# zhirui-gao/PoseProbe

Hardware: AMD Instinct MI355X
Metric: rays_per_sec_train_step (higher is better)
Workload: dtype f32 (3xf16-split products); 1 GPU; DTU-scan1-like 3-view 400x400, object-branch train step (ray select, render, losses, backward, TV+Adam), 160^3 grid, 186 samples/ray, N_rand=1024/GPU; per-step ray permutation + jitter pre-generated on the host and resident in HBM (the reference draws randperm inside the step); grid=160, n_rand_per_gpu=1024, samples_in_bbox_last_step=57637, parallelism=single GPU

## Files before the change

### poseprobe_amd/_lib.py

```python
import ctypes
import os
import re

HERE = os.path.dirname(os.path.abspath(__file__))
HEADER = os.path.join(HERE, '..', 'include', 'poseprobe_hip.h')
SO_PATH = os.path.join(HERE, 'libposeprobe_hip.so')


class pp_scene(ctypes.Structure):
    _fields_ = [('xyz_min', ctypes.c_float * 3), ('xyz_max', ctypes.c_float * 3), ('size', ctypes.c_int32 * 3),
                ('voxel_size', ctypes.c_float), ('stepsize', ctypes.c_float), ('near_clip', ctypes.c_float),
                ('far_clip', ctypes.c_float), ('bg', ctypes.c_float), ('n_samples', ctypes.c_int32),
                ('out_range', ctypes.c_float), ('k0_dim', ctypes.c_int32), ('pos_pe', ctypes.c_int32),
                ('view_pe', ctypes.c_int32), ('sdf_index_exact', ctypes.c_int32)]


def parse_header(path=HEADER):
    text = open(path).read()
    text = re.sub(r'/\*.*?\*/', '', text, flags=re.S)
    protos = {}
    for m in re.finditer(r'\bint\s+(pp_\w+)\s*\(([^;]*?)\)\s*;', text, flags=re.S):
        name, args = m.group(1), m.group(2)
        parsed = []
        for a in args.split(','):
            a = ' '.join(a.split())
            if a in ('void', ''):
                continue
            argname = re.findall(r'(\w+)$', a)[0]
            if 'pp_scene' in a:
                ct = ctypes.POINTER(pp_scene)
            elif 'char*' in a.replace(' *', '*'):
                ct = ctypes.c_char_p
            elif '*' in a:
                ct = ctypes.c_void_p
            elif 'uint8_t' in a and '*' not in a:
                ct = ctypes.c_uint8
            elif 'int64_t' in a:
                ct = ctypes.c_int64
            elif 'int32_t' in a or a.startswith('int '):
                ct = ctypes.c_int32
            elif 'float' in a:
                ct = ctypes.c_float
            else:
                raise ValueError(f'unhandled argument "{a}" in {name}')
            parsed.append((ct, argname))
        protos[name] = parsed
    return protos


class PoseProbeError(RuntimeError):
    pass


_lib = None


def lib():
    global _lib
    if _lib is not None:
        return _lib
    if not os.path.exists(SO_PATH):
        raise PoseProbeError(f'{SO_PATH} is missing: run `python -m poseprobe_amd.build_ext` '
                             '(there is no CPU / eager fallback for the hot path)')
    L = ctypes.CDLL(SO_PATH)
    L.pp_last_error.restype = ctypes.c_char_p
    L.pp_abi_version.restype = ctypes.c_int
    want = header_abi_version()
    if L.pp_abi_version() != want:
        raise PoseProbeError(f'{SO_PATH} reports ABI {L.pp_abi_version()}, include/poseprobe_hip.h declares {want}: '
                             'rebuild with `python -m poseprobe_amd.build_ext`')
    for name, args in parse_header().items():
        fn = getattr(L, name)
        fn.restype = ctypes.c_int
        fn.argtypes = [ct for ct, _ in args]
    _lib = L
    return L


def header_abi_version(path=HEADER):
    return int(re.search(r'#define\s+PP_ABI_VERSION\s+(\d+)', open(path).read()).group(1))


OPTION_NAMES = ('mlp_fused', 'grid_chunks', 'nerf_split', 'mlp_split', 'mlp_wgs', 'nerf_chain', 'nerf_chain_nw',
                'nerf_chain_head', 'mlp_pack', 'warp_lean')


class Context:

    def __init__(self, **options):
        self.handle = ctypes.c_void_p()
        check(lib().pp_context_create(ctypes.byref(self.handle)), 'pp_context_create')
        for k, v in options.items():
            self.set(k, v)

    def set(self, name, value):
        check(lib().pp_context_set_option(self.handle, name.encode(), int(value)), 'pp_context_set_option')

    def get(self, name):
        v = ctypes.c_int32()
        check(lib().pp_context_get_option(self.handle, name.encode(), ctypes.byref(v)), 'pp_context_get_option')
        return v.value

    def options(self):
        return {k: self.get(k) for k in OPTION_NAMES}

    def __del__(self):
        try:
            if _lib is not None and self.handle:
                _lib.pp_context_destroy(self.handle)
        except Exception:
            pass


_default_ctx = None


def default_context():
    global _default_ctx
    if _default_ctx is None:
        c = Context()
        for name in OPTION_NAMES:
            v = os.environ.get('PP_' + name.upper())
            if v not in (None, ''):
                c.set(name, int(v))
        _default_ctx = c
    return _default_ctx


def handle(ctx):
    return (default_context() if ctx is None else ctx).handle


def set_option(name, value):
    default_context().set(name, value)


def get_option(name):
    return default_context().get(name)


def library_default(name):
    v = ctypes.c_int32()
    check(lib().pp_context_get_option(None, name.encode(), ctypes.byref(v)), 'pp_context_get_option')
    return v.value


def check(status, name):
    if status != 0:
        raise PoseProbeError(f'{name} failed ({status}): {lib().pp_last_error().decode()}')


def call(name, *args):
    check(getattr(lib(), name)(*args), name)
```

### poseprobe_amd/csrc/pp_common.h

```cpp
#pragma once
#include <hip/hip_runtime.h>
#include <stdint.h>
#include <stdio.h>
#include <string.h>

#include "../../include/poseprobe_hip.h"

#define PP_WAVE 64

void pp_set_error(const char* fmt, ...);

enum PPOption {
  PP_OPT_MLP_FUSED = 0,
  PP_OPT_GRID_CHUNKS,
  PP_OPT_NERF_SPLIT,
  PP_OPT_MLP_SPLIT,
  PP_OPT_MLP_WGS,
  PP_OPT_NERF_CHAIN,
  PP_OPT_NERF_CHAIN_NW,
  PP_OPT_NERF_CHAIN_HEAD,
  PP_OPT_MLP_PACK,
  PP_OPT_WARP_LEAN,
  PP_OPT_COUNT
};

struct PPContext {
  int opt[PP_OPT_COUNT];
  const float* pack;
  const float* pack_params[2];
  const float* lean_acts;
  const float* lean_scratch;
  const float* lean_params;
  float* ord;
  int ord_wgs, ord_cap, ord_rays;
  float* nerf_ord;
};

struct PPOptScope {
  const int* prev;
  explicit PPOptScope(const void* ctx);
  ~PPOptScope();
};
int pp_opt(int id);
int pp_num_cus();
bool pp_launch_tv_march(const float* p, int X, int Y, int Z, int C, float scale, const float* g_scalar, float* grad, float* tv_out,
                        hipStream_t st);

#define PP_REQUIRE(cond, msg)                                     \
  do {                                                            \
    if (!(cond)) {                                                \
      pp_set_error("%s: %s", __func__, msg);                      \
      return PP_ERR_INVALID_ARG;                                  \
    }                                                             \
  } while (0)

#define PP_CHECK_LAUNCH()                                                           \
  do {                                                                              \
    hipError_t e__ = hipGetLastError();                                             \
    if (e__ != hipSuccess) {                                                        \
      pp_set_error("%s: kernel launch failed: %s", __func__, hipGetErrorString(e__)); \
      return PP_ERR_LAUNCH;                                                         \
    }                                                                               \
  } while (0)

static inline hipStream_t pp_stream(void* s) { return reinterpret_cast<hipStream_t>(s); }
static inline int pp_div_up(int a, int b) { return (a + b - 1) / b; }

struct SceneDev {
  float mn[3], mx[3];
  int sz[3];
  float voxel, stepsize, near_, far_, bg;
  int S;
  float out_range;
  int C, Lp, Lv;
  int flat_f32;
};

static inline SceneDev pp_scene_dev(const pp_scene* s) {
  SceneDev d;
  for (int i = 0; i < 3; ++i) { d.mn[i] = s->xyz_min[i]; d.mx[i] = s->xyz_max[i]; d.sz[i] = s->size[i]; }
  d.voxel = s->voxel_size; d.stepsize = s->stepsize; d.near_ = s->near_clip; d.far_ = s->far_clip; d.bg = s->bg;
  d.S = s->n_samples; d.out_range = s->out_range; d.C = s->k0_dim; d.Lp = s->pos_pe; d.Lv = s->view_pe;
  d.flat_f32 = ((long long)s->size[0] * s->size[1] * s->size[2] > (1ll << 24)) && s->sdf_index_exact == 0;
  return d;
}

#ifdef __HIPCC__
__device__ __forceinline__ float pp_mul(float a, float b) { return __fmul_rn(a, b); }
__device__ __forceinline__ float pp_add(float a, float b) { return __fadd_rn(a, b); }
__device__ __forceinline__ float pp_sub(float a, float b) { return __fsub_rn(a, b); }
__device__ __forceinline__ float pp_div(float a, float b) { return __fdiv_rn(a, b); }

__device__ __forceinline__ float pp_sigmoid(float x) { return 1.0f / (1.0f + expf(-x)); }
__device__ __forceinline__ float pp_softplus10(float x) {
  float bx = 10.0f * x;
  return bx > 20.0f ? x : log1pf(expf(bx)) / 10.0f;
}
__device__ __forceinline__ float pp_dsoftplus10(float x) {
  float bx = 10.0f * x;
  return bx > 20.0f ? 1.0f : pp_sigmoid(bx);
}

__device__ __forceinline__ float pp_wave_sum(float v) {
#pragma unroll
  for (int o = 32; o > 0; o >>= 1) v += __shfl_xor(v, o, 64);
  return v;
}

__device__ __forceinline__ float pp_grid_u(float p, float mn, float mx, int size) {
  float t = pp_div(pp_sub(p, mn), pp_sub(mx, mn));
  float n = pp_sub(pp_mul(t, 2.0f), 1.0f);
  return pp_mul(pp_div(pp_add(n, 1.0f), 2.0f), (float)(size - 1));
}
#endif
```

### poseprobe_amd/csrc/pp_error.hip

```cpp
#include <stdarg.h>

#include "pp_common.h"

static thread_local char g_err[512] = "";

void pp_set_error(const char* fmt, ...) {
  va_list ap;
  va_start(ap, fmt);
  vsnprintf(g_err, sizeof(g_err), fmt, ap);
  va_end(ap);
}

extern "C" const char* pp_last_error(void) { return g_err; }
extern "C" int pp_abi_version(void) { return PP_ABI_VERSION; }

struct PPOptionDef { const char* name; int dflt, lo, hi; };
static const PPOptionDef g_opt_def[PP_OPT_COUNT] = {
    {"mlp_fused", 1, 0, 1},          {"grid_chunks", 0, 0, 4096},  {"nerf_split", 1, 0, 1},
    {"mlp_split", 31, 0, 31},        {"mlp_wgs", 0, 0, 4096},      {"nerf_chain", 3, 0, 3},
    {"nerf_chain_nw", 4, 4, 8},      {"nerf_chain_head", 1, 0, 1}, {"mlp_pack", 1, 0, 1},
    {"warp_lean", 1, 0, 1},
};
static const struct PPDefaults {
  int v[PP_OPT_COUNT];
  PPDefaults() { for (int i = 0; i < PP_OPT_COUNT; ++i) v[i] = g_opt_def[i].dflt; }
} g_defaults;

static thread_local const int* t_opts = nullptr;
PPOptScope::PPOptScope(const void* ctx) : prev(t_opts) { t_opts = ctx ? static_cast<const PPContext*>(ctx)->opt : g_defaults.v; }
PPOptScope::~PPOptScope() { t_opts = prev; }
int pp_opt(int id) { return (t_opts ? t_opts : g_defaults.v)[id]; }

int pp_num_cus() {
  static const int n = [] {
    int dev = 0, cus = 0;
    if (hipGetDevice(&dev) == hipSuccess && hipDeviceGetAttribute(&cus, hipDeviceAttributeMultiprocessorCount, dev) == hipSuccess &&
        cus > 0)
      return cus;
    return 256;
  }();
  return n;
}

static int opt_find(const char* name) {
  for (int i = 0; i < PP_OPT_COUNT; ++i) if (name && strcmp(name, g_opt_def[i].name) == 0) return i;
  return -1;
}

extern "C" int pp_context_create(void** ctx) {
  PP_REQUIRE(ctx, "null pointer");
  PPContext* c = new PPContext;
  for (int i = 0; i < PP_OPT_COUNT; ++i) c->opt[i] = g_opt_def[i].dflt;
  c->pack = nullptr;
  c->pack_params[0] = c->pack_params[1] = nullptr;
  c->lean_acts = c->lean_scratch = c->lean_params = nullptr;
  c->ord = nullptr;
  c->ord_wgs = c->ord_cap = c->ord_rays = 0;
  c->nerf_ord = nullptr;
  *ctx = c;
  return PP_OK;
}

extern "C" int pp_context_destroy(void* ctx) {
  if (!ctx) return PP_OK;
  delete static_cast<PPContext*>(ctx);
  return PP_OK;
}

extern "C" int pp_context_set_option(void* ctx, const char* name, int32_t value) {
  PP_REQUIRE(ctx, "null context (the compiled-in defaults cannot be changed: create a context)");
  const int i = opt_find(name);
  if (i < 0) { pp_set_error("pp_context_set_option: unknown option '%s'", name ? name : "(null)"); return PP_ERR_INVALID_ARG; }
  if (value < g_opt_def[i].lo || value > g_opt_def[i].hi) {
    pp_set_error("pp_context_set_option: %s = %d outside [%d, %d]", name, value, g_opt_def[i].lo, g_opt_def[i].hi);
    return PP_ERR_INVALID_ARG;
  }
  static_cast<PPContext*>(ctx)->opt[i] = value;
  return PP_OK;
}

extern "C" int pp_context_get_option(const void* ctx, const char* name, int32_t* value) {
  const int i = opt_find(name);
  if (i < 0 || !value) { pp_set_error("pp_context_get_option: unknown option '%s'", name ? name : "(null)"); return PP_ERR_INVALID_ARG; }
  *value = ctx ? static_cast<const PPContext*>(ctx)->opt[i] : g_opt_def[i].dflt;
  return PP_OK;
}
```

### poseprobe_amd/csrc/pp_mlp_split.hip

```cpp
#include "pp_common.h"
#include "pp_mlp_fused.h"
#include "pp_gemm_split.h"
#include "pp_split_image.h"
#include "pp_mlp_pack.h"
#include "pp_ordered.h"

typedef float f32x4 __attribute__((ext_vector_type(4)));

#define LDA 132
#define TILE_ROWS 64
#define LDH2 136
#define PLANE (TILE_ROWS * LDH2)
#define PP_WAIT_VMEM() do { __builtin_amdgcn_s_waitcnt(0x0F70); asm volatile("" ::: "memory"); } while (0)

namespace {

struct SplitW { pp_half8 h[8], l[8]; };

__device__ __forceinline__ float wave_max(float v) {
#pragma unroll
  for (int o = 32; o > 0; o >>= 1) v = fmaxf(v, __shfl_xor(v, o, 64));
  return v;
}
template <int CTRL>
__device__ __forceinline__ float dpp_f(float v) {
  return __int_as_float(__builtin_amdgcn_update_dpp(0, __float_as_int(v), CTRL, 0xf, 0xf, true));
}
__device__ __forceinline__ float row_max16(float v) {
  v = fmaxf(v, dpp_f<0xB1>(v));
  v = fmaxf(v, dpp_f<0x4E>(v));
  v = fmaxf(v, dpp_f<0x141>(v));
  v = fmaxf(v, dpp_f<0x140>(v));
  return v;
}
__device__ __forceinline__ float block_max(float v, float* red, int tid, int& phase) {
  float* set = red + 16 * (phase & 1);
  ++phase;
  v = row_max16(v);
  if ((tid & 15) == 0) set[tid >> 4] = v;
  __syncthreads();
  const float4 a = *reinterpret_cast<const float4*>(set), b = *reinterpret_cast<const float4*>(set + 4),
               c = *reinterpret_cast<const float4*>(set + 8), d = *reinterpret_cast<const float4*>(set + 12);
  return fmaxf(fmaxf(fmaxf(fmaxf(a.x, a.y), fmaxf(a.z, a.w)), fmaxf(fmaxf(b.x, b.y), fmaxf(b.z, b.w))),
               fmaxf(fmaxf(fmaxf(c.x, c.y), fmaxf(c.z, c.w)), fmaxf(fmaxf(d.x, d.y), fmaxf(d.z, d.w))));
}
__device__ __forceinline__ int scale_exp(float mx) {
  if (!(mx > 0.f) || !(mx < 3.0e38f)) return 0;
  int e;
  frexpf(mx, &e);
  return min(max(15 - e, -60), 60);
}
__device__ __forceinline__ float pow2(int e) { return ldexpf(1.f, e); }
__device__ __forceinline__ float tile_scale(float mx) { return pow2(scale_exp(mx)); }
__device__ __forceinline__ void split1(float x, _Float16& h, _Float16& l) {
  h = (_Float16)x;
  l = (_Float16)(x - (float)h);
}
__device__ __forceinline__ void split8(const float4& a, const float4& b, float s, pp_half8& h, pp_half8& l) {
  const float v[8] = {a.x * s, a.y * s, a.z * s, a.w * s, b.x * s, b.y * s, b.z * s, b.w * s};
#pragma unroll
  for (int i = 0; i < 8; ++i) {
    _Float16 hh, ll;
    split1(v[i], hh, ll);
    h[i] = hh; l[i] = ll;
  }
}
__device__ __forceinline__ float amax4(const float4& v) { return fmaxf(fmaxf(fabsf(v.x), fabsf(v.y)), fmaxf(fabsf(v.z), fabsf(v.w))); }
__device__ __forceinline__ float asum4(const float4& v) { return (fabsf(v.x) + fabsf(v.y)) + (fabsf(v.z) + fabsf(v.w)); }

__device__ __forceinline__ int load_w_rows_split(SplitW& w, float& l1, const float* __restrict__ W, int n, int lh, float* red,
                                                   int tid, int& phase) {
  float4 v[16];
  float mx = 0.f, sum = 0.f;
#pragma unroll
  for (int ks = 0; ks < 8; ++ks) {
    v[2 * ks] = *reinterpret_cast<const float4*>(W + (size_t)n * 128 + 16 * ks + 8 * lh);
    v[2 * ks + 1] = *reinterpret_cast<const float4*>(W + (size_t)n * 128 + 16 * ks + 8 * lh + 4);
    mx = fmaxf(mx, fmaxf(amax4(v[2 * ks]), amax4(v[2 * ks + 1])));
    sum += asum4(v[2 * ks]) + asum4(v[2 * ks + 1]);
  }
  sum += __shfl_xor(sum, 32, 64);
  const int e = scale_exp(block_max(mx, red, tid, phase));
  const float s = pow2(e);
  l1 = block_max(sum, red, tid, phase) * 1.0001f;
#pragma unroll
  for (int ks = 0; ks < 8; ++ks) split8(v[2 * ks], v[2 * ks + 1], s, w.h[ks], w.l[ks]);
  return e;
}

template <int KS>
__device__ __forceinline__ void load_w_packed(SplitW& w, const float* __restrict__ img, int tid) {
  const pp_half8* __restrict__ p = reinterpret_cast<const pp_half8*>(img) + tid;
#pragma unroll
  for (int ks = 0; ks < KS; ++ks) { w.h[ks] = p[(2 * ks) * 256]; w.l[ks] = p[(2 * ks + 1) * 256]; }
#pragma unroll
  for (int ks = KS; ks < 8; ++ks) { w.h[ks] = w.h[0]; w.l[ks] = w.l[0]; }
}
template <int KS>
__device__ __forceinline__ void store_w_packed(float* __restrict__ img, const SplitW& w, int tid) {
  pp_half8* __restrict__ p = reinterpret_cast<pp_half8*>(img) + tid;
#pragma unroll
  for (int ks = 0; ks < KS; ++ks) { p[(2 * ks) * 256] = w.h[ks]; p[(2 * ks + 1) * 256] = w.l[ks]; }
}
__device__ __forceinline__ int pk_int(const float* __restrict__ pack, int slot) { return __float_as_int(pack[PK_SCAL + slot]); }

struct NoHook { __device__ __forceinline__ void operator()(int) const {} };
template <int KS = 8, int LD = LDH2, int PL = PLANE, class Hook = NoHook>
__device__ __forceinline__ void mma_half(const _Float16* __restrict__ rows, const SplitW& w, f32x16& acc, int l31, int lh,
                                         Hook hook = Hook()) {
  const _Float16* p = rows + l31 * LD + 8 * lh;
  pp_half8 h = *reinterpret_cast<const pp_half8*>(p), l = *reinterpret_cast<const pp_half8*>(p + PL);
#pragma unroll
  for (int ks = 0; ks < KS; ++ks) {
    pp_half8 nh = h, nl = l;
    if (ks + 1 < KS) {
      nh = *reinterpret_cast<const pp_half8*>(p + 16 * (ks + 1));
      nl = *reinterpret_cast<const pp_half8*>(p + 16 * (ks + 1) + PL);
    }
    acc = __builtin_amdgcn_mfma_f32_32x32x16_f16(w.h[ks], l, acc, 0, 0, 0);
    acc = __builtin_amdgcn_mfma_f32_32x32x16_f16(w.l[ks], h, acc, 0, 0, 0);
    acc = __builtin_amdgcn_mfma_f32_32x32x16_f16(w.h[ks], h, acc, 0, 0, 0);
    h = nh; l = nl;
    hook(ks);
  }
}

__device__ __forceinline__ void zero16(f32x16& acc) {
#pragma unroll
  for (int i = 0; i < 16; ++i) acc[i] = 0.f;
}

typedef _Float16 half2_t __attribute__((ext_vector_type(2)));

template <int COLS, bool SPLIT>
struct HalfEpilogue {
  float4 b[4];
  float y[16];
  float p[16];
  unsigned h[8], l[8];
  float xmax;
  __device__ __forceinline__ void begin(const float* __restrict__ brow) {
    xmax = 0.f;
#pragma unroll
    for (int q = 0; q < 4; ++q) b[q] = *reinterpret_cast<const float4*>(brow + 8 * q);
  }
  __device__ __forceinline__ void step(int i, const f32x16& acc, float inv, float snext, bool ok, float* __restrict__ Crow,
                                       _Float16* __restrict__ Arow) {
    __builtin_amdgcn_sched_barrier(0);
    if (i == 0) {
#pragma unroll
      for (int q = 0; q < 4; ++q) {
        y[4 * q] = fmaf(acc[4 * q], inv, b[q].x); y[4 * q + 1] = fmaf(acc[4 * q + 1], inv, b[q].y);
        y[4 * q + 2] = fmaf(acc[4 * q + 2], inv, b[q].z); y[4 * q + 3] = fmaf(acc[4 * q + 3], inv, b[q].w);
      }
    } else if (i == 1) {
      if (COLS == 4) {
#pragma unroll
        for (int e = 0; e < 16; ++e)
          asm("v_mov_b32_dpp %0, %1 quad_perm:[0,0,0,0] row_mask:0xf bank_mask:0xf bound_ctrl:1" : "=v"(p[e]) : "v"(y[e]));
#pragma unroll
        for (int e = 0; e < 16; ++e) asm("v_ashrrev_i32 %0, 31, %1" : "=v"(p[e]) : "v"(p[e]));
      }
    } else if (i == 2) {
#pragma unroll
      for (int e = 0; e < 16; ++e) {
        if (COLS == 4) asm("v_bfi_b32 %0, %1, 0, %2" : "=v"(y[e]) : "v"(p[e]), "v"(y[e]));
        else y[e] = fmaxf(y[e], 0.f);
      }
    } else if (SPLIT && i == 3) {
#pragma unroll
      for (int e = 0; e < 16; ++e) p[e] = y[e] * snext;
#pragma unroll
      for (int k = 0; k < 8; ++k) {
        asm("v_cvt_pk_f16_f32 %0, %1, %2" : "=v"(h[k]) : "v"(p[2 * k]), "v"(p[2 * k + 1]));
        asm("v_max3_f32 %0, |%1|, |%2|, %0" : "+v"(xmax) : "v"(p[2 * k]), "v"(p[2 * k + 1]));
      }
    } else if (SPLIT && i == 4) {
#pragma unroll
      for (int k = 0; k < 8; ++k) asm("v_fma_mixlo_f16 %0, %1, -1.0, %2 op_sel_hi:[1,0,0]" : "=v"(l[k]) : "v"(h[k]), "v"(p[2 * k]));
#pragma unroll
      for (int k = 0; k < 8; ++k)
        asm("v_fma_mixhi_f16 %0, %1, -1.0, %2 op_sel:[1,0,0] op_sel_hi:[1,0,0]" : "+v"(l[k]) : "v"(h[k]), "v"(p[2 * k + 1]));
    } else if (i == 5) {
      if (SPLIT) {
#pragma unroll
        for (int q = 0; q < 4; ++q) {
          *reinterpret_cast<uint2*>(Arow + 8 * q) = make_uint2(h[2 * q], h[2 * q + 1]);
          *reinterpret_cast<uint2*>(Arow + 8 * q + PLANE) = make_uint2(l[2 * q], l[2 * q + 1]);
        }
      } else {
#pragma unroll
        for (int q = 0; q < 4; ++q)
          *reinterpret_cast<float4*>(reinterpret_cast<float*>(Arow) + 8 * q) = make_float4(y[4 * q], y[4 * q + 1], y[4 * q + 2], y[4 * q + 3]);
      }
    } else if (i == 6) {
      if (ok) {
#pragma unroll
        for (int q = 0; q < 4; ++q) *reinterpret_cast<float4*>(Crow + 8 * q) = make_float4(y[4 * q], y[4 * q + 1], y[4 * q + 2], y[4 * q + 3]);
      }
    }
    __builtin_amdgcn_sched_barrier(0);
  }
  __device__ __forceinline__ void all(const f32x16& acc, float inv, float snext, bool ok, float* __restrict__ Crow, _Float16* __restrict__ Arow) {
#pragma unroll
    for (int i = 0; i < 8; ++i) step(i, acc, inv, snext, ok, Crow, Arow);
  }
  __device__ __forceinline__ float vmax(float ninv) const { return xmax * ninv; }
};

__device__ __forceinline__ void slot_max(unsigned* slot, float v, int lane) {
  v = row_max16(v);
  if ((lane & 15) == 0) {
    const unsigned a = (unsigned)(size_t)(__attribute__((address_space(3))) unsigned*)slot;
    asm volatile("ds_max_u32 %0, %1" ::"v"(a), "v"(__float_as_uint(v)) : "memory");
  }
}
__device__ __forceinline__ float slot_get(const unsigned* slot) { return __uint_as_float(*slot); }

}

template <bool PACK, bool LEAN>
__global__ __launch_bounds__(256) void k_warp_fused_fwd_s(const float* __restrict__ params, const float* __restrict__ pts,
                                                          const int32_t* __restrict__ count, int capacity, float out_range,
                                                          float* __restrict__ acts, float* __restrict__ out,
                                                          const float* __restrict__ pack) {
  __shared__ __attribute__((aligned(16))) _Float16 At[2][2 * PLANE];
  __shared__ __attribute__((aligned(16))) float W4s[4 * LDA];
  __shared__ __attribute__((aligned(16))) float Red[4 * 64 * 4];
  __shared__ float Ps[2][52];
  __shared__ unsigned Mx[2][8];
  __shared__ __attribute__((aligned(16))) float red4[32];
  __shared__ __attribute__((aligned(16))) float Bs[4][128];
  static_assert(2 * PLANE * 2 >= TILE_ROWS * LDA * 4, "fp32 view must fit into a split tile");
  const int M = min(count[0], capacity);
  const int R = 4 * M;
  const int ntiles = (M + 15) >> 4;
  if ((int)blockIdx.x >= ntiles) return;
  const int tid = threadIdx.x, lane = tid & 63, wid = tid >> 6;
  const int l31 = lane & 31, lh = lane >> 5;
  const int col = wid * 32 + l31;
  const int fb = wid * 32 + 4 * lh;
  const bool primal = (l31 & 3) == 0;
  const size_t LS = (size_t)capacity * 4 * 128;

  SplitW w1, w2, w3;
  int phase = 0;
  float l1_1, l1_2, l1_3, b1mx, b2mx, w0l1, w0mx, b0mx;
  int ew1, ew2, ew3, ew0;
  if (PACK) {
    load_w_packed<8>(w1, pack + PK_WARP, tid);
    load_w_packed<8>(w2, pack + PK_WARP + PK_IMG, tid);
    load_w_packed<8>(w3, pack + PK_WARP + 2 * PK_IMG, tid);
    ew1 = pk_int(pack, PKW_EW1); ew2 = pk_int(pack, PKW_EW2); ew3 = pk_int(pack, PKW_EW3); ew0 = pk_int(pack, PKW_EW0);
    l1_1 = pack[PKW_L1_1]; l1_2 = pack[PKW_L1_2]; l1_3 = pack[PKW_L1_3];
    b1mx = pack[PKW_B1MX]; b2mx = pack[PKW_B2MX]; w0l1 = pack[PKW_W0L1]; w0mx = pack[PKW_W0MX]; b0mx = pack[PKW_B0MX];
  } else {
    ew1 = load_w_rows_split(w1, l1_1, params + WPF_W1, col, lh, red4, tid, phase);
    ew2 = load_w_rows_split(w2, l1_2, params + WPF_W2, col, lh, red4, tid, phase);
    ew3 = load_w_rows_split(w3, l1_3, params + WPF_W3, col, lh, red4, tid, phase);
  }
  if (tid < 128) { Bs[0][tid] = params[WPF_B1 + tid]; Bs[1][tid] = params[WPF_B2 + tid]; Bs[2][tid] = params[WPF_B3 + tid]; Bs[3][tid] = 0.f; }
  auto brow = [&](int l) -> const float* { return &Bs[primal ? l : 3][fb]; };
  if (!PACK) {
    b1mx = block_max(fabsf(params[WPF_B1 + col]), red4, tid, phase);
    b2mx = block_max(fabsf(params[WPF_B2 + col]), red4, tid, phase);
  }
  const float w0x = params[WPF_W0 + col * 3], w0y = params[WPF_W0 + col * 3 + 1], w0z = params[WPF_W0 + col * 3 + 2];
  const float b0 = params[WPF_B0 + col];
  if (!PACK) {
    w0l1 = block_max((fabsf(w0x) + fabsf(w0y)) + fabsf(w0z), red4, tid, phase) * 1.0001f;
    w0mx = block_max(fmaxf(fmaxf(fabsf(w0x), fabsf(w0y)), fabsf(w0z)), red4, tid, phase);
    b0mx = block_max(fabsf(b0), red4, tid, phase);
    ew0 = scale_exp(fmaxf(w0mx, b0mx));
  }
  pp_half8 a0h, a0l;
  {
    const float z = 0.f;
    const float4 wa = lh == 0 ? make_float4(w0x, w0y, w0z, b0) : make_float4(z, z, z, z);
    split8(wa, make_float4(z, z, z, z), pow2(ew0), a0h, a0l);
  }
  for (int i = tid; i < 512; i += 256) W4s[(i >> 7) * LDA + (i & 127)] = params[WPF_W4 + i];
  const float b4 = (((tid >> 2) & 3) == 0) ? params[WPF_B4 + (tid & 3)] : 0.f;
  auto park = [&](int slot, float p) {
    if (wid == 0) {
      const float m = row_max16(fabsf(p));
      if (lane < 48) Ps[slot][lane] = p;
      if ((lane & 15) == 0 && lane < 48) Ps[slot][48 + (lane >> 4)] = m;
    }
  };
  float pnext = 0.f;
  if (tid < 48 && (int)blockIdx.x * 48 + tid < M * 3) pnext = pts[blockIdx.x * 48 + tid];
  park(0, pnext);
  if (tid < 16) Mx[tid >> 3][tid & 7] = 0u;
  __builtin_amdgcn_s_waitcnt(0);
  __syncthreads();
  int par = 0;
  for (int tile = blockIdx.x; tile < ntiles; tile += gridDim.x, par ^= 1) {
    const int s0 = tile * 16, r0 = tile * TILE_ROWS;
    {
      const int nt = tile + gridDim.x;
      pnext = 0.f;
      if (tid < 48 && nt < ntiles && nt * 48 + tid < M * 3) pnext = pts[nt * 48 + tid];
    }
    const bool ok0 = acts != nullptr && r0 + l31 < R, ok1 = acts != nullptr && r0 + 32 + l31 < R;
    float* __restrict__ crow = acts + (acts != nullptr ? (size_t)(r0 + l31) * 128 + fb : 0);
    _Float16* const arow0 = &At[0][l31 * LDH2 + fb];
    _Float16* const arow1 = &At[1][l31 * LDH2 + fb];
    float* const frow1 = reinterpret_cast<float*>(At[1]) + l31 * LDA + fb;
    f32x16 acc0, acc1;
    const float pmx = fmaxf(fmaxf(Ps[par][48], Ps[par][49]), Ps[par][50]);
    const int ein = scale_exp(fmaxf(pmx, 1.f));
    const int e0 = scale_exp(fmaxf(fmaf(w0l1, pmx, b0mx), w0mx));
    const float sin = pow2(ein), sc0 = pow2(e0);
    auto layer0 = [&](int t, f32x16& acc) {
      const int sl = 8 * t + (l31 >> 2), c = l31 & 3;
      const bool valid = s0 + sl < M && lh == 0;
      const float px = Ps[par][sl * 3], py = Ps[par][sl * 3 + 1], pz = Ps[par][sl * 3 + 2];
      float4 x = make_float4(c == 0 ? px : (c == 1 ? 1.f : 0.f), c == 0 ? py : (c == 2 ? 1.f : 0.f),
                             c == 0 ? pz : (c == 3 ? 1.f : 0.f), c == 0 ? 1.f : 0.f);
      if (!valid) x = make_float4(0.f, 0.f, 0.f, 0.f);
      pp_half8 xh, xl;
      split8(x, make_float4(0.f, 0.f, 0.f, 0.f), sin, xh, xl);
      zero16(acc);
      acc = __builtin_amdgcn_mfma_f32_32x32x16_f16(a0h, xl, acc, 0, 0, 0);
      acc = __builtin_amdgcn_mfma_f32_32x32x16_f16(a0l, xh, acc, 0, 0, 0);
      acc = __builtin_amdgcn_mfma_f32_32x32x16_f16(a0h, xh, acc, 0, 0, 0);
    };
    layer0(0, acc0);
    layer0(1, acc1);
    const float inv0 = pow2(-(ein + ew0)), ninv0 = pow2(-e0);
    HalfEpilogue<4, true> ea;
    ea.begin(brow(3));
    ea.all(acc0, inv0, sc0, ok0 && (!LEAN || primal), crow, arow0);
    slot_max(&Mx[par][0], ea.vmax(ninv0), lane);
    __syncthreads();
    if (tid < 8) Mx[par ^ 1][tid] = 0u;
    zero16(acc0);
    ea.begin(brow(3));
    mma_half(&At[0][0], w1, acc0, l31, lh, [&](int ks) { ea.step(ks, acc1, inv0, sc0, ok1 && (!LEAN || primal), crow + 32 * 128, arow0 + 32 * LDH2); });
    slot_max(&Mx[par][1], ea.vmax(ninv0), lane);
    park(par ^ 1, pnext);
    __syncthreads();
    const int e10 = scale_exp(fmaf(slot_get(&Mx[par][0]), l1_1, b1mx));
    const float sc10 = pow2(e10), inv1 = pow2(-(e0 + ew1));
    zero16(acc1);
    ea.begin(brow(0));
    mma_half(&At[0][32 * LDH2], w1, acc1, l31, lh, [&](int ks) { ea.step(ks, acc0, inv1, sc10, ok0, crow + LS, arow1); });
    slot_max(&Mx[par][2], ea.vmax(pow2(-e10)), lane);
    __syncthreads();
    const int e11 = scale_exp(fmaf(slot_get(&Mx[par][1]), l1_1, b1mx));
    const float sc11 = pow2(e11);
    zero16(acc0);
    ea.begin(brow(0));
    mma_half(&At[1][0], w2, acc0, l31, lh, [&](int ks) { ea.step(ks, acc1, inv1, sc11, ok1, crow + LS + 32 * 128, arow1 + 32 * LDH2); });
    slot_max(&Mx[par][3], ea.vmax(pow2(-e11)), lane);
    __syncthreads();
    const int e20 = scale_exp(fmaf(slot_get(&Mx[par][2]), l1_2, b2mx));
    const float sc20 = pow2(e20), inv20 = pow2(-(e10 + ew2)), inv21 = pow2(-(e11 + ew2));
    zero16(acc1);
    ea.begin(brow(1));
    mma_half(&At[1][32 * LDH2], w2, acc1, l31, lh, [&](int ks) { ea.step(ks, acc0, inv20, sc20, ok0, crow + 2 * LS, arow0); });
    __syncthreads();
    const int e21 = scale_exp(fmaf(slot_get(&Mx[par][3]), l1_2, b2mx));
    const float sc21 = pow2(e21);
    zero16(acc0);
    ea.begin(brow(1));
    mma_half(&At[0][0], w3, acc0, l31, lh, [&](int ks) { ea.step(ks, acc1, inv21, sc21, ok1, crow + 2 * LS + 32 * 128, arow0 + 32 * LDH2); });
    __syncthreads();
    HalfEpilogue<4, false> ef;
    const float inv30 = pow2(-(e20 + ew3)), inv31 = pow2(-(e21 + ew3));
    zero16(acc1);
    ef.begin(brow(2));
    mma_half(&At[0][32 * LDH2], w3, acc1, l31, lh, [&](int ks) { ef.step(ks, acc0, inv30, 1.f, ok0, crow + 3 * LS, reinterpret_cast<_Float16*>(frow1)); });
    ef.begin(brow(2));
    ef.all(acc1, inv31, 1.f, ok1, crow + 3 * LS + 32 * 128, reinterpret_cast<_Float16*>(frow1 + 32 * LDA));
    __syncthreads();
    {
      const float* As1 = reinterpret_cast<const float*>(At[1]);
      const float* xr = &As1[lane * LDA + 32 * wid];
      const float* wr = &W4s[(lane & 3) * LDA + 32 * wid];
      float4 xv[8], wv[8];
#pragma unroll
      for (int g = 0; g < 8; ++g) {
        xv[g] = *reinterpret_cast<const float4*>(xr + 4 * g);
        wv[g] = *reinterpret_cast<const float4*>(wr + 4 * g);
      }
      f32x4 d0 = {0.f, 0.f, 0.f, 0.f}, d1 = d0;
#pragma unroll
      for (int g = 0; g < 8; ++g) {
        d0 = __builtin_amdgcn_mfma_f32_4x4x1f32(xv[g].x, wv[g].x, d0, 0, 0, 0);
        d1 = __builtin_amdgcn_mfma_f32_4x4x1f32(xv[g].y, wv[g].y, d1, 0, 0, 0);
        d0 = __builtin_amdgcn_mfma_f32_4x4x1f32(xv[g].z, wv[g].z, d0, 0, 0, 0);
        d1 = __builtin_amdgcn_mfma_f32_4x4x1f32(xv[g].w, wv[g].w, d1, 0, 0, 0);
      }
      *reinterpret_cast<float4*>(&Red[(wid * 64 + lane) * 4]) = make_float4(d0[0] + d1[0], d0[1] + d1[1], d0[2] + d1[2], d0[3] + d1[3]);
    }
    __syncthreads();
    {
      const int row = tid >> 2, o = tid & 3;
      const int idx = ((row >> 2) * 4 + o) * 4 + (row & 3);
      const float sum = (Red[idx] + Red[256 + idx]) + (Red[512 + idx] + Red[768 + idx]);
      if (r0 + row < R) out[(size_t)r0 * 4 + tid] = (sum + b4) * out_range;
    }
  }
}

template <class... P, class... A>
static void launch_pack_variant(void (*with_pack)(P...), void (*without)(P...), int grid, hipStream_t st, const float* pack, A... args) {
  hipLaunchKernelGGL(pack ? with_pack : without, dim3(grid), dim3(256), 0, st, args..., pack);
}

int pp_launch_warp_fused_fwd_s(const float* params, const float* pts, const int32_t* count, int capacity, float out_range,
                               float* acts, float* out, hipStream_t st, const float* pack, bool lean) {
  const int ntiles = pp_div_up(capacity, 16);
  const int grid = ntiles < PP_FUSED_WGS ? ntiles : PP_FUSED_WGS;
  if (lean)
    launch_pack_variant(k_warp_fused_fwd_s<true, true>, k_warp_fused_fwd_s<false, true>, grid, st, pack, params, pts, count, capacity, out_range, acts, out);
  else
    launch_pack_variant(k_warp_fused_fwd_s<true, false>, k_warp_fused_fwd_s<false, false>, grid, st, pack, params, pts, count, capacity, out_range, acts, out);
  return 0;
}

namespace {

__device__ __forceinline__ int load_w_cols_split(SplitW& w, float& l1, const float* __restrict__ W, int j, int lh, float* red, int tid, int& phase) {
  float4 v[16];
  float mx = 0.f, sum = 0.f;
#pragma unroll
  for (int ks = 0; ks < 8; ++ks) {
    const float* p = W + (size_t)(16 * ks + 8 * lh) * 128 + j;
    v[2 * ks] = make_float4(p[0], p[128], p[256], p[384]);
    v[2 * ks + 1] = make_float4(p[512], p[640], p[768], p[896]);
    mx = fmaxf(mx, fmaxf(amax4(v[2 * ks]), amax4(v[2 * ks + 1])));
    sum += asum4(v[2 * ks]) + asum4(v[2 * ks + 1]);
  }
  sum += __shfl_xor(sum, 32, 64);
  const int e = scale_exp(block_max(mx, red, tid, phase));
  const float s = pow2(e);
  l1 = block_max(sum, red, tid, phase) * 1.0001f;
#pragma unroll
  for (int ks = 0; ks < 8; ++ks) split8(v[2 * ks], v[2 * ks + 1], s, w.h[ks], w.l[ks]);
  return e;
}

template <bool SPLIT>
struct HalfEpilogueB {
  float4 g[4];
  float y[16], p[16];
  unsigned h[8], l[8];
  unsigned long long m[16];
  float xmax;
  __device__ __forceinline__ void begin(const float* __restrict__ grow) {
    xmax = 0.f;
#pragma unroll
    for (int q = 0; q < 4; ++q) g[q] = *reinterpret_cast<const float4*>(grow + 8 * q);
  }
  __device__ __forceinline__ void step(int i, const f32x16& acc, float inv, float snext, bool ok, float* __restrict__ Crow,
                                       _Float16* __restrict__ Arow) {
    __builtin_amdgcn_sched_barrier(0);
    if (i == 0) {
#pragma unroll
      for (int e = 0; e < 16; ++e) y[e] = acc[e] * inv;
    } else if (i == 1) {
#pragma unroll
      for (int q = 0; q < 4; ++q) {
        asm volatile("v_cmp_lt_f32_e64 %0, 0, %1" : "=s"(m[4 * q]) : "v"(g[q].x));
        asm volatile("v_cmp_lt_f32_e64 %0, 0, %1" : "=s"(m[4 * q + 1]) : "v"(g[q].y));
        asm volatile("v_cmp_lt_f32_e64 %0, 0, %1" : "=s"(m[4 * q + 2]) : "v"(g[q].z));
        asm volatile("v_cmp_lt_f32_e64 %0, 0, %1" : "=s"(m[4 * q + 3]) : "v"(g[q].w));
      }
    } else if (i == 2) {
#pragma unroll
      for (int e = 0; e < 16; ++e) asm volatile("v_cndmask_b32_e64 %0, 0, %1, %2" : "=v"(y[e]) : "v"(y[e]), "s"(m[e]));
    } else if (SPLIT && i == 3) {
#pragma unroll
      for (int e = 0; e < 16; ++e) p[e] = y[e] * snext;
#pragma unroll
      for (int k = 0; k < 8; ++k) {
        asm("v_cvt_pk_f16_f32 %0, %1, %2" : "=v"(h[k]) : "v"(p[2 * k]), "v"(p[2 * k + 1]));
        asm("v_max3_f32 %0, |%1|, |%2|, %0" : "+v"(xmax) : "v"(p[2 * k]), "v"(p[2 * k + 1]));
      }
    } else if (SPLIT && i == 4) {
#pragma unroll
      for (int k = 0; k < 8; ++k) asm("v_fma_mixlo_f16 %0, %1, -1.0, %2 op_sel_hi:[1,0,0]" : "=v"(l[k]) : "v"(h[k]), "v"(p[2 * k]));
#pragma unroll
      for (int k = 0; k < 8; ++k)
        asm("v_fma_mixhi_f16 %0, %1, -1.0, %2 op_sel:[1,0,0] op_sel_hi:[1,0,0]" : "+v"(l[k]) : "v"(h[k]), "v"(p[2 * k + 1]));
    } else if (i == 5) {
      if (SPLIT) {
#pragma unroll
        for (int q = 0; q < 4; ++q) {
          *reinterpret_cast<uint2*>(Arow + 8 * q) = make_uint2(h[2 * q], h[2 * q + 1]);
          *reinterpret_cast<uint2*>(Arow + 8 * q + PLANE) = make_uint2(l[2 * q], l[2 * q + 1]);
        }
      } else {
#pragma unroll
        for (int q = 0; q < 4; ++q)
          *reinterpret_cast<float4*>(reinterpret_cast<float*>(Arow) + 8 * q) = make_float4(y[4 * q], y[4 * q + 1], y[4 * q + 2], y[4 * q + 3]);
      }
    } else if (i == 6) {
      if (Crow != nullptr && ok) {
#pragma unroll
        for (int q = 0; q < 4; ++q) *reinterpret_cast<float4*>(Crow + 8 * q) = make_float4(y[4 * q], y[4 * q + 1], y[4 * q + 2], y[4 * q + 3]);
      }
    }
    __builtin_amdgcn_sched_barrier(0);
  }
  __device__ __forceinline__ void all(const f32x16& acc, float inv, float snext, bool ok, float* __restrict__ Crow, _Float16* __restrict__ Arow) {
#pragma unroll
    for (int i = 0; i < 8; ++i) step(i, acc, inv, snext, ok, Crow, Arow);
  }
  __device__ __forceinline__ float vmax(float ninv) const { return xmax * ninv; }
};

#define PP_GLOBAL_PTR(p) ((const __attribute__((address_space(1))) void*)(p))
#define PP_LDS_PTR(p) ((__attribute__((address_space(3))) void*)(p))

}

template <bool PACK, bool LEAN>
__global__ __launch_bounds__(256) void k_warp_fused_bwd_s(const float* __restrict__ params, const float* __restrict__ pts,
                                                          const float* __restrict__ acts, const float* __restrict__ out_grad,
                                                          const int32_t* __restrict__ count, int capacity, float out_range,
                                                          float* __restrict__ ybar, float* __restrict__ params_grad,
                                                          float* __restrict__ pts_grad, float* __restrict__ part,
                                                          const float* __restrict__ pack) {
  __shared__ __attribute__((aligned(16))) _Float16 At[2][2 * PLANE];
  __shared__ __attribute__((aligned(16))) float XS[TILE_ROWS * 128];
  __shared__ __attribute__((aligned(16))) float GT[2][16 * 128];
  __shared__ __attribute__((aligned(16))) float W0s[4 * LDA];
  __shared__ __attribute__((aligned(16))) float G[2][256];
  __shared__ __attribute__((aligned(16))) float Ps[2][64];
  __shared__ __attribute__((aligned(16))) float Red[4 * 64];
  __shared__ unsigned Mx[2][8];
  __shared__ __attribute__((aligned(16))) float red4[32];
  const int M = min(count[0], capacity);
  const int R = 4 * M;
  const int ntiles = (M + 15) >> 4;
  if ((int)blockIdx.x >= ntiles) return;
  const int tid = threadIdx.x, lane = tid & 63, wid = tid >> 6;
  const int l31 = lane & 31, lh = lane >> 5;
  const int col = wid * 32 + l31;
  const int fb = wid * 32 + 4 * lh;
  const int pr = l31 >> 2;
  const size_t LS = (size_t)capacity * 4 * 128;
  const float* __restrict__ X0 = acts;
  const float* __restrict__ X1 = acts + LS;
  const float* __restrict__ X2 = acts + 2 * LS;
  const float* __restrict__ X3 = acts + 3 * LS;

  SplitW w3, w2, w1;
  int phase = 0;
  float l1_3, l1_2, l1_1;
  int ew3, ew2, ew1;
  if (PACK) {
    load_w_packed<8>(w3, pack + PK_WARP + 3 * PK_IMG, tid);
    load_w_packed<8>(w2, pack + PK_WARP + 4 * PK_IMG, tid);
    load_w_packed<8>(w1, pack + PK_WARP + 5 * PK_IMG, tid);
    ew3 = pk_int(pack, PKW_EW3C); ew2 = pk_int(pack, PKW_EW2C); ew1 = pk_int(pack, PKW_EW1C);
    l1_3 = pack[PKW_L1_3C]; l1_2 = pack[PKW_L1_2C]; l1_1 = pack[PKW_L1_1C];
  } else {
    ew3 = load_w_cols_split(w3, l1_3, params + WPF_W3, col, lh, red4, tid, phase);
    ew2 = load_w_cols_split(w2, l1_2, params + WPF_W2, col, lh, red4, tid, phase);
    ew1 = load_w_cols_split(w1, l1_1, params + WPF_W1, col, lh, red4, tid, phase);
  }
  const float w4a = params[WPF_W4 + col] * out_range, w4b = params[WPF_W4 + 128 + col] * out_range,
              w4c = params[WPF_W4 + 256 + col] * out_range, w4d = params[WPF_W4 + 384 + col] * out_range;
  const float w4l1 = block_max((fabsf(w4a) + fabsf(w4b)) + (fabsf(w4c) + fabsf(w4d)), red4, tid, phase) * 1.0001f;
  const int ew4 = scale_exp(block_max(fmaxf(fmaxf(fabsf(w4a), fabsf(w4b)), fmaxf(fabsf(w4c), fabsf(w4d))), red4, tid, phase));
  pp_half8 a4h, a4l;
  {
    const float z = 0.f;
    const float4 wa = lh == 0 ? make_float4(w4a, w4b, w4c, w4d) : make_float4(z, z, z, z);
    split8(wa, make_float4(z, z, z, z), pow2(ew4), a4h, a4l);
  }
  const int j0 = tid & 127, h0 = tid >> 7;
  for (int i = tid; i < 512; i += 256) {
    const int r = i >> 7, j = i & 127;
    W0s[r * LDA + j] = (r < 3) ? params[WPF_W0 + j * 3 + r] : 0.f;
  }
  float wacc4[4] = {0.f, 0.f, 0.f, 0.f}, bacc4 = 0.f, wacc0[3] = {0.f, 0.f, 0.f}, bacc0 = 0.f;

  auto stage_piece = [&](int t, int b, int i) {
    const int rn0 = t * TILE_ROWS, sn0 = t * 16;
    if (i < 8) {
      const int rl = 16 * wid + 2 * i;
      const int row = min(rn0 + rl + lh, R - 1);
      __builtin_amdgcn_global_load_lds(PP_GLOBAL_PTR(X3 + (size_t)row * 128 + l31 * 4), PP_LDS_PTR(&XS[rl * 128]), 16, 0, 0);
    } else if (i == 8) {
      const int e = min(sn0 * 16 + tid, M * 16 - 1);
      __builtin_amdgcn_global_load_lds(PP_GLOBAL_PTR(out_grad + e), PP_LDS_PTR(&G[b][wid * 64]), 4, 0, 0);
    } else if (wid == 0) {
      const int e = min(sn0 * 3 + lane, M * 3 - 1);
      __builtin_amdgcn_global_load_lds(PP_GLOBAL_PTR(pts + e), PP_LDS_PTR(&Ps[b][0]), 4, 0, 0);
    }
  };
  auto stage_gate_piece = [&](const float* __restrict__ X, int r0, int gb, int i) {
    const int prow = 4 * wid + 2 * i;
    const int row = min(r0 + 4 * (prow + lh), R - 1);
    __builtin_amdgcn_global_load_lds(PP_GLOBAL_PTR(X + (size_t)row * 128 + l31 * 4), PP_LDS_PTR(&GT[gb][prow * 128]), 16, 0, 0);
  };
  auto prepare_grad = [&](int t, int b) {
    float gv = G[b][tid];
    if (t * 16 + (tid >> 4) >= M) { gv = 0.f; G[b][tid] = 0.f; }
    slot_max(&Mx[b][6], fabsf(gv), lane);
  };
  auto w4_accumulate = [&](int b) {
    const float* __restrict__ xs = &XS[(h0 * 32) * 128 + j0];
#pragma unroll 8
    for (int r = 0; r < 32; ++r) {
      const float4 gq = *reinterpret_cast<const float4*>(&G[b][(h0 * 32 + r) * 4]);
      const float x = xs[r * 128];
      wacc4[0] = fmaf(gq.x, x, wacc4[0]); wacc4[1] = fmaf(gq.y, x, wacc4[1]);
      wacc4[2] = fmaf(gq.z, x, wacc4[2]); wacc4[3] = fmaf(gq.w, x, wacc4[3]);
      if (j0 < 4 && (r & 3) == 0) bacc4 += G[b][(h0 * 32 + r) * 4 + j0];
    }
  };
  auto out_layer = [&](int b, int t, float sg, f32x16& acc) {
    float4 x = *reinterpret_cast<const float4*>(&G[b][(t * 32 + l31) * 4]);
    if (lh != 0) x = make_float4(0.f, 0.f, 0.f, 0.f);
    pp_half8 xh, xl;
    split8(x, make_float4(0.f, 0.f, 0.f, 0.f), sg, xh, xl);
    zero16(acc);
    acc = __builtin_amdgcn_mfma_f32_32x32x16_f16(a4h, xl, acc, 0, 0, 0);
    acc = __builtin_amdgcn_mfma_f32_32x32x16_f16(a4l, xh, acc, 0, 0, 0);
    acc = __builtin_amdgcn_mfma_f32_32x32x16_f16(a4h, xh, acc, 0, 0, 0);
  };
  int e3n0 = 0, e3n1 = 0;
  auto out_layer_bwd = [&](int t, int b) {
    const float gmx = slot_get(&Mx[b][6]);
    const int eg = scale_exp(gmx);
    const int e3 = scale_exp(gmx * w4l1);
    const float sg = pow2(eg), s3 = pow2(e3), inv = pow2(-(eg + ew4)), n3 = pow2(-e3);
    const int r0 = t * TILE_ROWS;
    f32x16 a0, a1;
    out_layer(b, 0, sg, a0);
    out_layer(b, 1, sg, a1);
    HalfEpilogueB<true> eb;
    float* crow = LEAN ? nullptr : ybar + (size_t)(r0 + l31) * 128 + fb;
    if (LEAN && t * 16 + (tid >> 4) < M) ybar[(size_t)t * 256 + tid] = G[b][tid] * out_range;
    eb.begin(&XS[(4 * pr) * 128 + fb]);
    eb.all(a0, inv, s3, r0 + l31 < R, crow, &At[0][l31 * LDH2 + fb]);
    slot_max(&Mx[b][0], eb.vmax(n3), lane);
    eb.begin(&XS[(32 + 4 * pr) * 128 + fb]);
    eb.all(a1, inv, s3, r0 + 32 + l31 < R, LEAN ? nullptr : crow + 32 * 128, &At[0][(32 + l31) * LDH2 + fb]);
    slot_max(&Mx[b][1], eb.vmax(n3), lane);
    e3n0 = e3; e3n1 = e3;
  };

  if (tid < 16) Mx[tid >> 3][tid & 7] = 0u;
#pragma unroll
  for (int i = 0; i < 10; ++i) stage_piece(blockIdx.x, 0, i);
  __builtin_amdgcn_s_waitcnt(0);
  __syncthreads();
  prepare_grad(blockIdx.x, 0);
  __syncthreads();
  w4_accumulate(0);
  out_layer_bwd(blockIdx.x, 0);
  __syncthreads();

  int par = 0;
  for (int tile = blockIdx.x; tile < ntiles; tile += gridDim.x, par ^= 1) {
    const int r0 = tile * TILE_ROWS, s0 = tile * 16;
    const int tnext = tile + gridDim.x;
    const bool more = tnext < ntiles;
    const bool ok0 = r0 + l31 < R, ok1 = r0 + 32 + l31 < R;
    const int e30 = e3n0, e31 = e3n1;
    float* const crow = ybar + (size_t)(r0 + l31) * 128 + fb;
    _Float16* const arow0 = &At[0][l31 * LDH2 + fb];
    _Float16* const arow1 = &At[1][l31 * LDH2 + fb];
    float* const frow1 = reinterpret_cast<float*>(At[1]) + l31 * LDA + fb;
    const float* const grow0 = &GT[0][pr * 128 + fb];
    const float* const grow1 = &GT[1][pr * 128 + fb];
    f32x16 acc0, acc1;
    HalfEpilogueB<true> eb;
    if (tid < 7) Mx[par ^ 1][tid] = 0u;
    zero16(acc0);
    mma_half(&At[0][0], w3, acc0, l31, lh, [&](int ks) {
      if (ks < 2) stage_gate_piece(X2, r0, 0, ks);
      if (more) { stage_piece(tnext, par ^ 1, ks); if (ks < 2) stage_piece(tnext, par ^ 1, 8 + ks); }
    });
    PP_WAIT_VMEM();
    __syncthreads();
    const int e20 = scale_exp(slot_get(&Mx[par][0]) * l1_3), e21 = scale_exp(slot_get(&Mx[par][1]) * l1_3);
    if (more) prepare_grad(tnext, par ^ 1);
    zero16(acc1);
    eb.begin(grow0);
    mma_half(&At[0][32 * LDH2], w3, acc1, l31, lh, [&](int ks) {
      eb.step(ks, acc0, pow2(-(e30 + ew3)), pow2(e20), ok0, crow + LS, arow1);
      if (ks == 7) { stage_gate_piece(X1, r0, 1, 0); stage_gate_piece(X1, r0, 1, 1); }
    });
    slot_max(&Mx[par][2], eb.vmax(pow2(-e20)), lane);
    __syncthreads();
    zero16(acc0);
    eb.begin(grow0 + 8 * 128);
    mma_half(&At[1][0], w2, acc0, l31, lh, [&](int ks) {
      if (ks == 5) PP_WAIT_VMEM();
      eb.step(ks, acc1, pow2(-(e31 + ew3)), pow2(e21), ok1, crow + LS + 32 * 128, arow1 + 32 * LDH2);
    });
    slot_max(&Mx[par][3], eb.vmax(pow2(-e21)), lane);
    __syncthreads();
    const int e10 = scale_exp(slot_get(&Mx[par][2]) * l1_2), e11 = scale_exp(slot_get(&Mx[par][3]) * l1_2);
    zero16(acc1);
    eb.begin(grow1);
    mma_half(&At[1][32 * LDH2], w2, acc1, l31, lh, [&](int ks) {
      eb.step(ks, acc0, pow2(-(e20 + ew2)), pow2(e10), ok0, crow + 2 * LS, arow0);
      if (ks == 7) { stage_gate_piece(X0, r0, 0, 0); stage_gate_piece(X0, r0, 0, 1); }
    });
    __syncthreads();
    zero16(acc0);
    eb.begin(grow1 + 8 * 128);
    mma_half(&At[0][0], w1, acc0, l31, lh, [&](int ks) {
      if (ks == 5) PP_WAIT_VMEM();
      eb.step(ks, acc1, pow2(-(e21 + ew2)), pow2(e11), ok1, crow + 2 * LS + 32 * 128, arow0 + 32 * LDH2);
    });
    __syncthreads();
    HalfEpilogueB<false> ef;
    zero16(acc1);
    ef.begin(grow0);
    mma_half(&At[0][32 * LDH2], w1, acc1, l31, lh, [&](int ks) {
      ef.step(ks, acc0, pow2(-(e10 + ew1)), 1.f, false, nullptr, reinterpret_cast<_Float16*>(frow1));
    });
    ef.begin(grow0 + 8 * 128);
    ef.all(acc1, pow2(-(e11 + ew1)), 1.f, false, nullptr, reinterpret_cast<_Float16*>(frow1 + 32 * LDA));
    __syncthreads();
    const float* As1 = reinterpret_cast<const float*>(At[1]);
    {
      const float* __restrict__ yb = &As1[(4 * h0 * 8) * LDA + j0];
      const float* ps = &Ps[par][h0 * 24];
#pragma unroll
      for (int q = 0; q < 8; ++q) {
        const float y0 = yb[(4 * q) * LDA], y1 = yb[(4 * q + 1) * LDA], y2 = yb[(4 * q + 2) * LDA], y3 = yb[(4 * q + 3) * LDA];
        wacc0[0] += y0 * ps[q * 3] + y1;
        wacc0[1] += y0 * ps[q * 3 + 1] + y2;
        wacc0[2] += y0 * ps[q * 3 + 2] + y3;
        bacc0 += y0;
      }
    }
    {
      const float* xr = &As1[lane * LDA + 32 * wid];
      const float* wr = &W0s[(lane & 3) * LDA + 32 * wid];
      float4 xv[8], wv[8];
#pragma unroll
      for (int g = 0; g < 8; ++g) {
        xv[g] = *reinterpret_cast<const float4*>(xr + 4 * g);
        wv[g] = *reinterpret_cast<const float4*>(wr + 4 * g);
      }
      f32x4 d0 = {0.f, 0.f, 0.f, 0.f}, d1 = d0;
#pragma unroll
      for (int g = 0; g < 8; ++g) {
        d0 = __builtin_amdgcn_mfma_f32_4x4x1f32(xv[g].x, wv[g].x, d0, 0, 0, 0);
        d1 = __builtin_amdgcn_mfma_f32_4x4x1f32(xv[g].y, wv[g].y, d1, 0, 0, 0);
        d0 = __builtin_amdgcn_mfma_f32_4x4x1f32(xv[g].z, wv[g].z, d0, 0, 0, 0);
        d1 = __builtin_amdgcn_mfma_f32_4x4x1f32(xv[g].w, wv[g].w, d1, 0, 0, 0);
      }
      Red[wid * 64 + lane] = d0[0] + d1[0];
    }
    if (more) {
      w4_accumulate(par ^ 1);
      out_layer_bwd(tnext, par ^ 1);
    }
    __syncthreads();
    if (tid < 64) {
      const int s = tid >> 2, i = tid & 3;
      if (i < 3 && s0 + s < M) {
        const float v = (Red[tid] + Red[64 + tid]) + (Red[128 + tid] + Red[192 + tid]);
        atomicAdd(&pts_grad[(s0 + s) * 3 + i], v);
      }
    }
  }

  __syncthreads();
  float* red = reinterpret_cast<float*>(At[0]);
  if (h0 == 1) {
#pragma unroll
    for (int o = 0; o < 4; ++o) red[o * 128 + j0] = wacc4[o];
#pragma unroll
    for (int i = 0; i < 3; ++i) red[(4 + i) * 128 + j0] = wacc0[i];
    red[7 * 128 + j0] = bacc0;
    if (j0 < 4) red[8 * 128 + j0] = bacc4;
  }
  __syncthreads();
  if (h0 == 0 && part != nullptr) {
    float* __restrict__ row = part + (size_t)blockIdx.x * ORD_WARP_THIN;
#pragma unroll
    for (int o = 0; o < 4; ++o) row[o * 128 + j0] = (wacc4[o] + red[o * 128 + j0]) * out_range;
#pragma unroll
    for (int i = 0; i < 3; ++i) row[512 + j0 * 3 + i] = wacc0[i] + red[(4 + i) * 128 + j0];
    row[896 + j0] = bacc0 + red[7 * 128 + j0];
    if (j0 < 4) row[1024 + j0] = (bacc4 + red[8 * 128 + j0]) * out_range;
  } else if (h0 == 0) {
#pragma unroll
    for (int o = 0; o < 4; ++o) atomicAdd(&params_grad[WPF_W4 + o * 128 + j0], (wacc4[o] + red[o * 128 + j0]) * out_range);
#pragma unroll
    for (int i = 0; i < 3; ++i) atomicAdd(&params_grad[WPF_W0 + j0 * 3 + i], wacc0[i] + red[(4 + i) * 128 + j0]);
    atomicAdd(&params_grad[WPF_B0 + j0], bacc0 + red[7 * 128 + j0]);
    if (j0 < 4) atomicAdd(&params_grad[WPF_B4 + j0], (bacc4 + red[8 * 128 + j0]) * out_range);
  }
}

int pp_launch_warp_fused_bwd_s(const float* params, const float* pts, const float* acts, const float* out_grad,
                               const int32_t* count, int capacity, float out_range, float* ybar, float* params_grad,
                               float* pts_grad, hipStream_t st, const float* pack, float* part, bool lean) {
  const int ntiles = pp_div_up(capacity, 16);
  const int grid = ntiles < PP_FUSED_WGS ? ntiles : PP_FUSED_WGS;
  if (lean)
    launch_pack_variant(k_warp_fused_bwd_s<true, true>, k_warp_fused_bwd_s<false, true>, grid, st, pack, params, pts, acts, out_grad, count,
                        capacity, out_range, ybar, params_grad, pts_grad, part);
  else
    launch_pack_variant(k_warp_fused_bwd_s<true, false>, k_warp_fused_bwd_s<false, false>, grid, st, pack, params, pts, acts, out_grad, count,
                        capacity, out_range, ybar, params_grad, pts_grad, part);
  if (part) {
    const OrdSegs segs{4, {512, 896, 1024, ORD_WARP_THIN_N}, {WPF_W4, WPF_W0, WPF_B0, WPF_B4}};
    pp_launch_ordered_flush(part, ORD_WARP_THIN, grid, count, capacity, 16, segs, params_grad, st);
  }
  return 0;
}

namespace {

#define FLD 72
#define FPL (TILE_ROWS * FLD)

__device__ __forceinline__ int load_w0_rows_split(SplitW& w, float& l1, const float* __restrict__ W, int n, int lh, float* red, int tid, int& phase) {
  float4 v[8];
  float mx = 0.f, sum = 0.f;
#pragma unroll
  for (int ks = 0; ks < 4; ++ks) {
    v[2 * ks] = *reinterpret_cast<const float4*>(W + (size_t)n * 64 + 16 * ks + 8 * lh);
    v[2 * ks + 1] = *reinterpret_cast<const float4*>(W + (size_t)n * 64 + 16 * ks + 8 * lh + 4);
    mx = fmaxf(mx, fmaxf(amax4(v[2 * ks]), amax4(v[2 * ks + 1])));
    sum += asum4(v[2 * ks]) + asum4(v[2 * ks + 1]);
  }
  sum += __shfl_xor(sum, 32, 64);
  const int e = scale_exp(block_max(mx, red, tid, phase));
  const float s = pow2(e);
  l1 = block_max(sum, red, tid, phase) * 1.0001f;
#pragma unroll
  for (int ks = 0; ks < 4; ++ks) split8(v[2 * ks], v[2 * ks + 1], s, w.h[ks], w.l[ks]);
#pragma unroll
  for (int ks = 4; ks < 8; ++ks) { w.h[ks] = w.h[0]; w.l[ks] = w.l[0]; }
  return e;
}

__device__ __forceinline__ int load_w0_cols_split(SplitW& w, const float* __restrict__ W, int f, int lh, float* red, int tid, int& phase) {
  float4 v[16];
  float mx = 0.f;
#pragma unroll
  for (int ks = 0; ks < 8; ++ks) {
    const float* p = W + (size_t)(16 * ks + 8 * lh) * 64 + f;
    v[2 * ks] = make_float4(p[0], p[64], p[128], p[192]);
    v[2 * ks + 1] = make_float4(p[256], p[320], p[384], p[448]);
    mx = fmaxf(mx, fmaxf(amax4(v[2 * ks]), amax4(v[2 * ks + 1])));
  }
  const int e = scale_exp(block_max(mx, red, tid, phase));
  const float s = pow2(e);
#pragma unroll
  for (int ks = 0; ks < 8; ++ks) split8(v[2 * ks], v[2 * ks + 1], s, w.h[ks], w.l[ks]);
  return e;
}

__device__ __forceinline__ void stage_feat_tile_s(const float* __restrict__ feat, int r0, int R, float* Fs, int wid, int lane) {
#pragma unroll
  for (int i = 0; i < 4; ++i) {
    const int rl = 16 * wid + 4 * i + (lane >> 4);
    const int c4 = (lane & 15) ^ (rl & 15);
    const int row = min(r0 + rl, R - 1);
    __builtin_amdgcn_global_load_lds(PP_GLOBAL_PTR(feat + (size_t)row * 64 + c4 * 4), PP_LDS_PTR(Fs + (16 * wid + 4 * i) * 64), 16, 0, 0);
  }
}

}

template <bool PACK>
__global__ __launch_bounds__(256) void k_rgb_fused_fwd_s(const float* __restrict__ params, const float* __restrict__ feat,
                                                         const int32_t* __restrict__ count, int capacity,
                                                         const float* __restrict__ logit_add, int add_ld,
                                                         float* __restrict__ acts, float* __restrict__ rgb,
                                                         const float* __restrict__ pack) {
  __shared__ __attribute__((aligned(16))) _Float16 At[2][2 * PLANE];
  __shared__ __attribute__((aligned(16))) float Fs[2][TILE_ROWS * 64];
  __shared__ __attribute__((aligned(16))) _Float16 Fh[2 * FPL];
  __shared__ __attribute__((aligned(16))) float W3s[4 * LDA];
  __shared__ __attribute__((aligned(16))) float Red[4 * 64 * 4];
  __shared__ __attribute__((aligned(16))) float Bs[3][128];
  __shared__ int Er[TILE_ROWS];
  __shared__ unsigned Mx[2][8];
  __shared__ __attribute__((aligned(16))) float red4[32];
  const int R = min(count[0], capacity);
  const int ntiles = (R + TILE_ROWS - 1) / TILE_ROWS;
  if ((int)blockIdx.x >= ntiles) return;
  const int tid = threadIdx.x, lane = tid & 63, wid = tid >> 6;
  const int l31 = lane & 31, lh = lane >> 5;
  const int col = wid * 32 + l31;
  const int fb = wid * 32 + 4 * lh;
  const size_t LS = (size_t)capacity * 128;

  SplitW w0, w1, w2;
  int phase = 0;
  float l1_0, l1_1, l1_2, b0mx, b1mx;
  int ew0, ew1, ew2;
  if (PACK) {
    load_w_packed<4>(w0, pack + PK_RGB, tid);
    load_w_packed<8>(w1, pack + PK_RGB_W1, tid);
    load_w_packed<8>(w2, pack + PK_RGB_W1 + PK_IMG, tid);
    ew0 = pk_int(pack, PKR_EW0); ew1 = pk_int(pack, PKR_EW1); ew2 = pk_int(pack, PKR_EW2);
    l1_0 = pack[PKR_L1_0]; l1_1 = pack[PKR_L1_1]; l1_2 = pack[PKR_L1_2];
    b0mx = pack[PKR_B0MX]; b1mx = pack[PKR_B1MX];
  } else {
    ew0 = load_w0_rows_split(w0, l1_0, params + RGF_W0, col, lh, red4, tid, phase);
    ew1 = load_w_rows_split(w1, l1_1, params + RGF_W1, col, lh, red4, tid, phase);
    ew2 = load_w_rows_split(w2, l1_2, params + RGF_W2, col, lh, red4, tid, phase);
    b0mx = block_max(fabsf(params[RGF_B0 + col]), red4, tid, phase);
    b1mx = block_max(fabsf(params[RGF_B1 + col]), red4, tid, phase);
  }
  if (tid < 128) { Bs[0][tid] = params[RGF_B0 + tid]; Bs[1][tid] = params[RGF_B1 + tid]; Bs[2][tid] = params[RGF_B2 + tid]; }
  for (int i = tid; i < 512; i += 256) {
    const int r = i >> 7, j = i & 127;
    W3s[r * LDA + j] = (r < 3) ? params[RGF_W3 + r * 128 + j] : 0.f;
  }
  const float b3 = ((tid & 3) < 3) ? params[RGF_B3 + (tid & 3)] : 0.f;
  if (tid < 16) Mx[tid >> 3][tid & 7] = 0u;
  stage_feat_tile_s(feat, blockIdx.x * TILE_ROWS, R, Fs[0], wid, lane);
  __builtin_amdgcn_s_waitcnt(0);
  __syncthreads();

  int par = 0;
  for (int tile = blockIdx.x; tile < ntiles; tile += gridDim.x, par ^= 1) {
    const int r0 = tile * TILE_ROWS;
    const int tnext = tile + gridDim.x;
    const bool ok0 = acts != nullptr && r0 + l31 < R, ok1 = acts != nullptr && r0 + 32 + l31 < R;
    float* __restrict__ crow = acts + (acts != nullptr ? (size_t)(r0 + l31) * 128 + fb : 0);
    _Float16* const arow0 = &At[0][l31 * LDH2 + fb];
    _Float16* const arow1 = &At[1][l31 * LDH2 + fb];
    float* const frow0 = reinterpret_cast<float*>(At[0]) + l31 * LDA + fb;
    PP_WAIT_VMEM();
    {
      const int row = tid >> 2, qd = tid & 3;
      float4 f[4];
#pragma unroll
      for (int i = 0; i < 4; ++i) f[i] = *reinterpret_cast<const float4*>(&Fs[par][row * 64 + (((4 * qd + i) ^ (row & 15)) << 2)]);
      float mx = fmaxf(fmaxf(amax4(f[0]), amax4(f[1])), fmaxf(amax4(f[2]), amax4(f[3])));
      if (r0 + row >= R) { mx = 0.f; f[0] = f[1] = f[2] = f[3] = make_float4(0.f, 0.f, 0.f, 0.f); }
      mx = fmaxf(mx, dpp_f<0xB1>(mx));
      mx = fmaxf(mx, dpp_f<0x4E>(mx));
      const int er = scale_exp(mx);
      const float sr = pow2(er);
      pp_half8 h0, l0, h1, l1;
      split8(f[0], f[1], sr, h0, l0);
      split8(f[2], f[3], sr, h1, l1);
      _Float16* d = &Fh[row * FLD + 16 * qd];
      *reinterpret_cast<pp_half8*>(d) = h0; *reinterpret_cast<pp_half8*>(d + 8) = h1;
      *reinterpret_cast<pp_half8*>(d + FPL) = l0; *reinterpret_cast<pp_half8*>(d + FPL + 8) = l1;
      if (qd == 0) Er[row] = er;
      slot_max(&Mx[par][wid >> 1], mx, lane);
    }
    if (tnext < ntiles) stage_feat_tile_s(feat, tnext * TILE_ROWS, R, Fs[par ^ 1], wid, lane);
    __syncthreads();
    if (tid < 6) Mx[par ^ 1][tid] = 0u;
    f32x16 acc0, acc1;
    HalfEpilogue<1, true> ea;
    const int e00 = scale_exp(fmaf(slot_get(&Mx[par][0]), l1_0, b0mx)), e01 = scale_exp(fmaf(slot_get(&Mx[par][1]), l1_0, b0mx));
    const float inv00 = pow2(-(Er[l31] + ew0)), inv01 = pow2(-(Er[32 + l31] + ew0));
    zero16(acc0);
    mma_half<4, FLD, FPL>(&Fh[0], w0, acc0, l31, lh);
    zero16(acc1);
    ea.begin(&Bs[0][fb]);
    mma_half<4, FLD, FPL>(&Fh[32 * FLD], w0, acc1, l31, lh, [&](int ks) {
      ea.step(2 * ks, acc0, inv00, pow2(e00), ok0, crow, arow0);
      ea.step(2 * ks + 1, acc0, inv00, pow2(e00), ok0, crow, arow0);
    });
    slot_max(&Mx[par][2], ea.vmax(pow2(-e00)), lane);
    __syncthreads();
    zero16(acc0);
    ea.begin(&Bs[0][fb]);
    mma_half(&At[0][0], w1, acc0, l31, lh, [&](int ks) { ea.step(ks, acc1, inv01, pow2(e01), ok1, crow + 32 * 128, arow0 + 32 * LDH2); });
    slot_max(&Mx[par][3], ea.vmax(pow2(-e01)), lane);
    __syncthreads();
    const int e10 = scale_exp(fmaf(slot_get(&Mx[par][2]), l1_1, b1mx));
    zero16(acc1);
    ea.begin(&Bs[1][fb]);
    mma_half(&At[0][32 * LDH2], w1, acc1, l31, lh, [&](int ks) { ea.step(ks, acc0, pow2(-(e00 + ew1)), pow2(e10), ok0, crow + LS, arow1); });
    __syncthreads();
    const int e11 = scale_exp(fmaf(slot_get(&Mx[par][3]), l1_1, b1mx));
    zero16(acc0);
    ea.begin(&Bs[1][fb]);
    mma_half(&At[1][0], w2, acc0, l31, lh, [&](int ks) { ea.step(ks, acc1, pow2(-(e01 + ew1)), pow2(e11), ok1, crow + LS + 32 * 128, arow1 + 32 * LDH2); });
    __syncthreads();
    HalfEpilogue<1, false> ef;
    zero16(acc1);
    ef.begin(&Bs[2][fb]);
    mma_half(&At[1][32 * LDH2], w2, acc1, l31, lh, [&](int ks) { ef.step(ks, acc0, pow2(-(e10 + ew2)), 1.f, ok0, crow + 2 * LS, reinterpret_cast<_Float16*>(frow0)); });
    ef.begin(&Bs[2][fb]);
    ef.all(acc1, pow2(-(e11 + ew2)), 1.f, ok1, crow + 2 * LS + 32 * 128, reinterpret_cast<_Float16*>(frow0 + 32 * LDA));
    __syncthreads();
    {
      const float* As0 = reinterpret_cast<const float*>(At[0]);
      const float* xr = &As0[lane * LDA + 32 * wid];
      const float* wr = &W3s[(lane & 3) * LDA + 32 * wid];
      float4 xv[8], wv[8];
#pragma unroll
      for (int g = 0; g < 8; ++g) {
        xv[g] = *reinterpret_cast<const float4*>(xr + 4 * g);
        wv[g] = *reinterpret_cast<const float4*>(wr + 4 * g);
      }
      f32x4 d0 = {0.f, 0.f, 0.f, 0.f}, d1 = d0;
#pragma unroll
      for (int g = 0; g < 8; ++g) {
        d0 = __builtin_amdgcn_mfma_f32_4x4x1f32(xv[g].x, wv[g].x, d0, 0, 0, 0);
        d1 = __builtin_amdgcn_mfma_f32_4x4x1f32(xv[g].y, wv[g].y, d1, 0, 0, 0);
        d0 = __builtin_amdgcn_mfma_f32_4x4x1f32(xv[g].z, wv[g].z, d0, 0, 0, 0);
        d1 = __builtin_amdgcn_mfma_f32_4x4x1f32(xv[g].w, wv[g].w, d1, 0, 0, 0);
      }
      *reinterpret_cast<float4*>(&Red[(wid * 64 + lane) * 4]) = make_float4(d0[0] + d1[0], d0[1] + d1[1], d0[2] + d1[2], d0[3] + d1[3]);
    }
    __syncthreads();
    {
      const int row = tid >> 2, o = tid & 3;
      const int idx = ((row >> 2) * 4 + o) * 4 + (row & 3);
      const float sum = (Red[idx] + Red[256 + idx]) + (Red[512 + idx] + Red[768 + idx]);
      if (o < 3 && r0 + row < R) {
        const size_t m = (size_t)(r0 + row);
        rgb[m * 3 + o] = pp_sigmoid(sum + b3 + (logit_add ? logit_add[m * add_ld + o] : 0.f));
      }
    }
  }
}

int pp_launch_rgb_fused_fwd_s(const float* params, const float* feat, const int32_t* count, int capacity,
                              const float* logit_add, int add_ld, float* acts, float* rgb, hipStream_t st, const float* pack) {
  const int ntiles = pp_div_up(capacity, TILE_ROWS);
  const int grid = ntiles < PP_FUSED_WGS ? ntiles : PP_FUSED_WGS;
  launch_pack_variant(k_rgb_fused_fwd_s<true>, k_rgb_fused_fwd_s<false>, grid, st, pack, params, feat, count, capacity, logit_add, add_ld, acts, rgb);
  return 0;
}

template <bool PACK>
__global__ __launch_bounds__(256) void k_rgb_fused_bwd_s(const float* __restrict__ params, const float* __restrict__ acts,
                                                         const float* __restrict__ rgb, const float* __restrict__ rgb_grad,
                                                         const int32_t* __restrict__ count, int capacity,
                                                         float* __restrict__ ybar, float* __restrict__ params_grad,
                                                         float* __restrict__ feat_grad, float* __restrict__ logit_grad, int lg_ld,
                                                         float* __restrict__ part, const float* __restrict__ pack) {
  __shared__ __attribute__((aligned(16))) _Float16 At[2][2 * PLANE];
  __shared__ __attribute__((aligned(16))) float XS[TILE_ROWS * 128];
  __shared__ __attribute__((aligned(16))) float GT[TILE_ROWS * 128];
  __shared__ __attribute__((aligned(16))) float RG[2][2][192];
  __shared__ __attribute__((aligned(16))) float GL[TILE_ROWS * 4];
  __shared__ unsigned Mx[2][8];
  __shared__ __attribute__((aligned(16))) float red4[32];
  const int R = min(count[0], capacity);
  const int ntiles = (R + TILE_ROWS - 1) / TILE_ROWS;
  if ((int)blockIdx.x >= ntiles) return;
  const int tid = threadIdx.x, lane = tid & 63, wid = tid >> 6;
  const int l31 = lane & 31, lh = lane >> 5;
  const int col = wid * 32 + l31;
  const int fb = wid * 32 + 4 * lh;
  const size_t LS = (size_t)capacity * 128;
  const float* __restrict__ H0 = acts;
  const float* __restrict__ H1 = acts + LS;
  const float* __restrict__ H2 = acts + 2 * LS;

  SplitW w2, w1, w0;
  int phase = 0;
  float l1_2, l1_1;
  const int rb = wid >> 1, fcol = (wid & 1) * 32 + l31;
  const float w3a = params[RGF_W3 + col], w3b = params[RGF_W3 + 128 + col], w3c = params[RGF_W3 + 256 + col];
  int ew2, ew1, ew0, ew3;
  float w3l1;
  if (PACK) {
    load_w_packed<8>(w2, pack + PK_RGB_W1 + 2 * PK_IMG, tid);
    load_w_packed<8>(w1, pack + PK_RGB_W1 + 3 * PK_IMG, tid);
    load_w_packed<8>(w0, pack + PK_RGB_W1 + 4 * PK_IMG, tid);
    ew2 = pk_int(pack, PKR_EW2C); ew1 = pk_int(pack, PKR_EW1C); ew0 = pk_int(pack, PKR_EW0T); ew3 = pk_int(pack, PKR_EW3);
    l1_2 = pack[PKR_L1_2C]; l1_1 = pack[PKR_L1_1C]; w3l1 = pack[PKR_W3L1];
  } else {
    ew2 = load_w_cols_split(w2, l1_2, params + RGF_W2, col, lh, red4, tid, phase);
    ew1 = load_w_cols_split(w1, l1_1, params + RGF_W1, col, lh, red4, tid, phase);
    ew0 = load_w0_cols_split(w0, params + RGF_W0, fcol, lh, red4, tid, phase);
    w3l1 = block_max((fabsf(w3a) + fabsf(w3b)) + fabsf(w3c), red4, tid, phase) * 1.0001f;
    ew3 = scale_exp(block_max(fmaxf(fmaxf(fabsf(w3a), fabsf(w3b)), fabsf(w3c)), red4, tid, phase));
  }
  pp_half8 a3h, a3l;
  {
    const float z = 0.f;
    const float4 wa = lh == 0 ? make_float4(w3a, w3b, w3c, z) : make_float4(z, z, z, z);
    split8(wa, make_float4(z, z, z, z), pow2(ew3), a3h, a3l);
  }
  const int j0 = tid & 127, h0 = tid >> 7;
  float wacc3[3] = {0.f, 0.f, 0.f}, bacc3 = 0.f;

  auto stage_tile = [&](const float* __restrict__ X, int r0, float* dst) {
#pragma unroll
    for (int i = 0; i < 8; ++i) {
      const int rl = 16 * wid + 2 * i;
      const int row = min(r0 + rl + lh, R - 1);
      __builtin_amdgcn_global_load_lds(PP_GLOBAL_PTR(X + (size_t)row * 128 + l31 * 4), PP_LDS_PTR(dst + rl * 128), 16, 0, 0);
    }
  };
  auto stage = [&](int t, int b) {
    const int r0 = t * TILE_ROWS;
    stage_tile(H2, r0, XS);
    if (wid < 3) {
      const int e = min(r0 * 3 + tid, R * 3 - 1);
      __builtin_amdgcn_global_load_lds(PP_GLOBAL_PTR(rgb + e), PP_LDS_PTR(&RG[b][0][wid * 64]), 4, 0, 0);
      __builtin_amdgcn_global_load_lds(PP_GLOBAL_PTR(rgb_grad + e), PP_LDS_PTR(&RG[b][1][wid * 64]), 4, 0, 0);
    }
  };
  auto logit_grads = [&](int t, int b) {
    const int r0 = t * TILE_ROWS;
    float gl = 0.f;
    if (tid < 192) {
      const int m = tid / 3, o = tid - 3 * m;
      const float r = RG[b][0][tid];
      gl = (r0 + m < R) ? RG[b][1][tid] * r * (1.f - r) : 0.f;
      GL[m * 4 + o] = gl;
      if (logit_grad && r0 + m < R) logit_grad[(size_t)(r0 + m) * lg_ld + o] = gl;
    } else {
      GL[(tid - 192) * 4 + 3] = 0.f;
    }
    slot_max(&Mx[b][4], fabsf(gl), lane);
  };
  auto w3_accumulate = [&]() {
    const float* __restrict__ xs = &XS[(h0 * 32) * 128 + j0];
#pragma unroll 8
    for (int r = 0; r < 32; ++r) {
      const float4 g = *reinterpret_cast<const float4*>(&GL[(h0 * 32 + r) * 4]);
      const float x = xs[r * 128];
      wacc3[0] = fmaf(g.x, x, wacc3[0]); wacc3[1] = fmaf(g.y, x, wacc3[1]); wacc3[2] = fmaf(g.z, x, wacc3[2]);
      if (j0 < 3) bacc3 += GL[(h0 * 32 + r) * 4 + j0];
    }
  };
  int e2n = 0;
  auto out_layer_bwd = [&](int t, int b, _Float16* dst) {
    const float gmx = slot_get(&Mx[b][4]);
    const int eg = scale_exp(gmx);
    const int e2 = scale_exp(gmx * w3l1);
    const float sg = pow2(eg), s2 = pow2(e2), inv = pow2(-(eg + ew3)), n2 = pow2(-e2);
    const int r0 = t * TILE_ROWS;
    float* crow = ybar + (size_t)(r0 + l31) * 128 + fb;
    HalfEpilogueB<true> eb;
#pragma unroll
    for (int hh = 0; hh < 2; ++hh) {
      float4 x = *reinterpret_cast<const float4*>(&GL[(hh * 32 + l31) * 4]);
      if (lh != 0) x = make_float4(0.f, 0.f, 0.f, 0.f);
      pp_half8 xh, xl;
      split8(x, make_float4(0.f, 0.f, 0.f, 0.f), sg, xh, xl);
      f32x16 a;
      zero16(a);
      a = __builtin_amdgcn_mfma_f32_32x32x16_f16(a3h, xl, a, 0, 0, 0);
      a = __builtin_amdgcn_mfma_f32_32x32x16_f16(a3l, xh, a, 0, 0, 0);
      a = __builtin_amdgcn_mfma_f32_32x32x16_f16(a3h, xh, a, 0, 0, 0);
      eb.begin(&XS[(hh * 32 + l31) * 128 + fb]);
      eb.all(a, inv, s2, r0 + hh * 32 + l31 < R, crow + hh * 32 * 128, dst + (hh * 32 + l31) * LDH2 + fb);
      slot_max(&Mx[b][hh], eb.vmax(n2), lane);
    }
    e2n = e2;
  };

  if (tid < 16) Mx[tid >> 3][tid & 7] = 0u;
  stage(blockIdx.x, 0);
  __builtin_amdgcn_s_waitcnt(0);
  __syncthreads();
  logit_grads(blockIdx.x, 0);
  __syncthreads();
  w3_accumulate();
  out_layer_bwd(blockIdx.x, 0, At[0]);
  __syncthreads();

  int par = 0;
  for (int tile = blockIdx.x; tile < ntiles; tile += gridDim.x, par ^= 1) {
    const int r0 = tile * TILE_ROWS;
    const int tnext = tile + gridDim.x;
    const bool more = tnext < ntiles;
    const bool ok0 = r0 + l31 < R, ok1 = r0 + 32 + l31 < R;
    _Float16* const Aa = At[par];
    _Float16* const Ab = At[par ^ 1];
    const int e2 = e2n;
    float* const crow = ybar + (size_t)(r0 + l31) * 128 + fb;
    f32x16 acc0, acc1;
    HalfEpilogueB<true> eb;
    if (tid < 5) Mx[par ^ 1][tid] = 0u;
    if (more) stage(tnext, par ^ 1);
    stage_tile(H1, r0, GT);
    zero16(acc0);
    mma_half(Aa, w2, acc0, l31, lh);
    PP_WAIT_VMEM();
    __syncthreads();
    const int e10 = scale_exp(slot_get(&Mx[par][0]) * l1_2), e11 = scale_exp(slot_get(&Mx[par][1]) * l1_2);
    zero16(acc1);
    eb.begin(&GT[l31 * 128 + fb]);
    mma_half(Aa + 32 * LDH2, w2, acc1, l31, lh, [&](int ks) {
      eb.step(ks, acc0, pow2(-(e2 + ew2)), pow2(e10), ok0, crow + LS, Ab + l31 * LDH2 + fb);
    });
    slot_max(&Mx[par][2], eb.vmax(pow2(-e10)), lane);
    __syncthreads();
    zero16(acc0);
    eb.begin(&GT[(32 + l31) * 128 + fb]);
    mma_half(Ab, w1, acc0, l31, lh, [&](int ks) {
      eb.step(ks, acc1, pow2(-(e2 + ew2)), pow2(e11), ok1, crow + LS + 32 * 128, Ab + (32 + l31) * LDH2 + fb);
    });
    slot_max(&Mx[par][3], eb.vmax(pow2(-e11)), lane);
    __syncthreads();
    stage_tile(H0, r0, GT);
    zero16(acc1);
    mma_half(Ab + 32 * LDH2, w1, acc1, l31, lh);
    PP_WAIT_VMEM();
    __syncthreads();
    const int e00 = scale_exp(slot_get(&Mx[par][2]) * l1_1), e01 = scale_exp(slot_get(&Mx[par][3]) * l1_1);
    eb.begin(&GT[l31 * 128 + fb]);
    eb.all(acc0, pow2(-(e10 + ew1)), pow2(e00), ok0, crow + 2 * LS, Aa + l31 * LDH2 + fb);
    eb.begin(&GT[(32 + l31) * 128 + fb]);
    eb.all(acc1, pow2(-(e11 + ew1)), pow2(e01), ok1, crow + 2 * LS + 32 * 128, Aa + (32 + l31) * LDH2 + fb);
    if (more) logit_grads(tnext, par ^ 1);
    __syncthreads();
    {
      f32x16 fa;
      zero16(fa);
      mma_half(Aa + rb * 32 * LDH2, w0, fa, l31, lh);
      const float inv = pow2(-((rb ? e01 : e00) + ew0));
      const int row = r0 + rb * 32 + l31;
      if (row < R) {
        float* __restrict__ ft = feat_grad + (size_t)row * 64 + (wid & 1) * 32 + 4 * lh;
#pragma unroll
        for (int q = 0; q < 4; ++q)
          *reinterpret_cast<float4*>(ft + 8 * q) = make_float4(fa[4 * q] * inv, fa[4 * q + 1] * inv, fa[4 * q + 2] * inv, fa[4 * q + 3] * inv);
      }
    }
    if (more) {
      w3_accumulate();
      out_layer_bwd(tnext, par ^ 1, Ab);
    }
    __syncthreads();
  }

  float* red = reinterpret_cast<float*>(At[0]);
  __syncthreads();
  if (h0 == 1) {
#pragma unroll
    for (int o = 0; o < 3; ++o) red[o * 128 + j0] = wacc3[o];
    if (j0 < 3) red[4 * 128 + j0] = bacc3;
  }
  __syncthreads();
  if (h0 == 0 && part != nullptr) {
    float* __restrict__ row = part + (size_t)blockIdx.x * ORD_RGB_THIN;
#pragma unroll
    for (int o = 0; o < 3; ++o) row[o * 128 + j0] = wacc3[o] + red[o * 128 + j0];
    if (j0 < 3) row[384 + j0] = bacc3 + red[4 * 128 + j0];
  } else if (h0 == 0) {
#pragma unroll
    for (int o = 0; o < 3; ++o) atomicAdd(&params_grad[RGF_W3 + o * 128 + j0], wacc3[o] + red[o * 128 + j0]);
    if (j0 < 3) atomicAdd(&params_grad[RGF_B3 + j0], bacc3 + red[4 * 128 + j0]);
  }
}

int pp_launch_rgb_fused_bwd_s(const float* params, const float* acts, const float* rgb, const float* rgb_grad,
                              const int32_t* count, int capacity, float* ybar, float* params_grad, float* feat_grad,
                              float* logit_grad, int lg_ld, hipStream_t st, const float* pack, float* part) {
  const int ntiles = pp_div_up(capacity, TILE_ROWS);
  const int grid = ntiles < PP_FUSED_WGS ? ntiles : PP_FUSED_WGS;
  launch_pack_variant(k_rgb_fused_bwd_s<true>, k_rgb_fused_bwd_s<false>, grid, st, pack, params, acts, rgb, rgb_grad, count, capacity, ybar,
                      params_grad, feat_grad, logit_grad, lg_ld, part);
  if (part) {
    const OrdSegs segs{2, {384, ORD_RGB_THIN_N, 0, 0}, {RGF_W3, RGF_B3, 0, 0}};
    pp_launch_ordered_flush(part, ORD_RGB_THIN, grid, count, capacity, TILE_ROWS, segs, params_grad, st);
  }
  return 0;
}

__global__ __launch_bounds__(256) void k_mlp_pack(const float* __restrict__ warp, const float* __restrict__ rgb, float* __restrict__ pack) {
  __shared__ __attribute__((aligned(16))) float red4[32];
  const int task = blockIdx.x;
  const float* __restrict__ params = task < PK_TASKS_WARP ? warp : rgb;
  if (params == nullptr) return;
  const int tid = threadIdx.x, lane = tid & 63, wid = tid >> 6;
  const int l31 = lane & 31, lh = lane >> 5;
  const int col = wid * 32 + l31;
  int phase = 0;
  SplitW w;
  float l1 = 0.f;
  float* __restrict__ S = pack + PK_SCAL;
  auto put = [&](int se, int e, int sl, float v) {
    if (tid == 0) { S[se] = __int_as_float(e); if (sl >= 0) S[sl] = v; }
  };
  if (task < 3) {
    const int off = task == 0 ? WPF_W1 : (task == 1 ? WPF_W2 : WPF_W3);
    const int e = load_w_rows_split(w, l1, params + off, col, lh, red4, tid, phase);
    store_w_packed<8>(pack + PK_WARP + task * PK_IMG, w, tid);
    put(PKW_EW1 + 2 * task, e, PKW_L1_1 + 2 * task, l1);
  } else if (task < 6) {
    const int t = task - 3;
    const int off = t == 0 ? WPF_W3 : (t == 1 ? WPF_W2 : WPF_W1);
    const int e = load_w_cols_split(w, l1, params + off, col, lh, red4, tid, phase);
    store_w_packed<8>(pack + PK_WARP + task * PK_IMG, w, tid);
    put(PKW_EW3C + 2 * t, e, PKW_L1_3C + 2 * t, l1);
  } else if (task == 6) {
    const float b1mx = block_max(fabsf(params[WPF_B1 + col]), red4, tid, phase), b2mx = block_max(fabsf(params[WPF_B2 + col]), red4, tid, phase);
    const float w0x = params[WPF_W0 + col * 3], w0y = params[WPF_W0 + col * 3 + 1], w0z = params[WPF_W0 + col * 3 + 2];
    const float b0 = params[WPF_B0 + col];
    const float w0l1 = block_max((fabsf(w0x) + fabsf(w0y)) + fabsf(w0z), red4, tid, phase) * 1.0001f;
    const float w0mx = block_max(fmaxf(fmaxf(fabsf(w0x), fabsf(w0y)), fabsf(w0z)), red4, tid, phase);
    const float b0mx = block_max(fabsf(b0), red4, tid, phase);
    if (tid == 0) { S[PKW_B1MX] = b1mx; S[PKW_B2MX] = b2mx; S[PKW_W0L1] = w0l1; S[PKW_W0MX] = w0mx; S[PKW_B0MX] = b0mx; }
    put(PKW_EW0, scale_exp(fmaxf(w0mx, b0mx)), -1, 0.f);
  } else if (task == 7) {
    const int e = load_w0_rows_split(w, l1, params + RGF_W0, col, lh, red4, tid, phase);
    store_w_packed<4>(pack + PK_RGB, w, tid);
    put(PKR_EW0, e, PKR_L1_0, l1);
  } else if (task < 10) {
    const int t = task - 8;
    const int e = load_w_rows_split(w, l1, params + (t == 0 ? RGF_W1 : RGF_W2), col, lh, red4, tid, phase);
    store_w_packed<8>(pack + PK_RGB_W1 + t * PK_IMG, w, tid);
    put(PKR_EW1 + 2 * t, e, PKR_L1_1 + 2 * t, l1);
  } else if (task < 12) {
    const int t = task - 10;
    const int e = load_w_cols_split(w, l1, params + (t == 0 ? RGF_W2 : RGF_W1), col, lh, red4, tid, phase);
    store_w_packed<8>(pack + PK_RGB_W1 + (2 + t) * PK_IMG, w, tid);
    put(PKR_EW2C + 2 * t, e, PKR_L1_2C + 2 * t, l1);
  } else if (task == 12) {
    const int e = load_w0_cols_split(w, params + RGF_W0, (wid & 1) * 32 + l31, lh, red4, tid, phase);
    store_w_packed<8>(pack + PK_RGB_W1 + 4 * PK_IMG, w, tid);
    put(PKR_EW0T, e, -1, 0.f);
  } else {
    const float b0mx = block_max(fabsf(params[RGF_B0 + col]), red4, tid, phase), b1mx = block_max(fabsf(params[RGF_B1 + col]), red4, tid, phase);
    const float w3a = params[RGF_W3 + col], w3b = params[RGF_W3 + 128 + col], w3c = params[RGF_W3 + 256 + col];
    const float w3l1 = block_max((fabsf(w3a) + fabsf(w3b)) + fabsf(w3c), red4, tid, phase) * 1.0001f;
    const int ew3 = scale_exp(block_max(fmaxf(fmaxf(fabsf(w3a), fabsf(w3b)), fabsf(w3c)), red4, tid, phase));
    if (tid == 0) { S[PKR_B0MX] = b0mx; S[PKR_B1MX] = b1mx; }
    put(PKR_EW3, ew3, PKR_W3L1, w3l1);
  }
}

int pp_launch_mlp_pack(const float* warp_params, const float* rgbnet_params, float* pack, hipStream_t st) {
  hipLaunchKernelGGL(k_mlp_pack, dim3(PK_TASKS), dim3(256), 0, st, warp_params, rgbnet_params, pack);
  return 0;
}

namespace {

struct WgsUnit { int r0, rend; };

__device__ __forceinline__ WgsUnit wgs_unit(int k, int full, int wg, int nwg, int ntiles, int R, int rem_rows, int q) {
  if (k < full) {
    const int t = ntiles - 1 - wg - k * nwg;
    return {t * TILE_ROWS, R};
  }
  const int hi = rem_rows - wg * q;
  return {max(hi - q, 0), hi};
}

__device__ __forceinline__ void wgs_active(int ntiles, int& nwg_ab, int& nwg_c) {
  if (ntiles < 8 * nwg_ab) {
    nwg_ab = max(nwg_ab / 2, 1);
    nwg_c = max(nwg_c / 2, 1);
  }
}

template <int KX, int CSTEP, bool LEAN>
__device__ __forceinline__ void wgs_layer(const WgradOperands& L, const float* __restrict__ gate3, const float* __restrict__ wls,
                                          int layer, int R, int ntiles, int wg, int nwg, unsigned char* __restrict__ img,
                                          float2* __restrict__ flags, float* __restrict__ slot) {
  static_assert(!LEAN || KX == 128, "the lean form is the warp net's");
  constexpr int NB = KX / 64;
  constexpr int XR = KX / 16;
  constexpr int XC = KX / 4;
  const int full = ntiles / nwg;
  const int rem_rows = min((ntiles - full * nwg) * TILE_ROWS, R);
  const int q = ((rem_rows + nwg - 1) / nwg + 15) & ~15;
  const int nunits = full + (rem_rows - wg * q > 0 ? 1 : 0);
  if (nunits == 0) {
    if (slot != nullptr)
      for (int i = threadIdx.x; i < ORD_WGRAD_SLOT / 4; i += 256) reinterpret_cast<float4*>(slot)[i] = make_float4(0.f, 0.f, 0.f, 0.f);
    return;
  }
  unsigned char* const Yh = img;
  unsigned char* const Yl = img + TILE_ROWS * 256;
  unsigned char* const Xh = img + 2 * TILE_ROWS * 256;
  unsigned char* const Xl = img + 3 * TILE_ROWS * 256;
  const int tid = threadIdx.x, lane = tid & 63, wid = tid >> 6;
  const int wr = wid >> 1, wc = wid & 1, l31 = lane & 31, lh = lane >> 5;
  const int c4 = tid & 31, rblk = tid >> 5;
  const int xc4 = c4 % XC, xrow = 8 * rblk + (c4 / XC) * XR;
  const bool bias = L.bbar != nullptr;
  const bool lean_y = LEAN && layer == 0, lean_x = LEAN && layer == 2;
  float4 rg[2];
  f32x16 acc[2][NB];
#pragma unroll
  for (int t = 0; t < 2; ++t)
#pragma unroll
    for (int u = 0; u < NB; ++u) zero16(acc[t][u]);
  float bsum[4] = {0.f, 0.f, 0.f, 0.f};
  int eY = 60, eX = 60;
  float sY = pow2(eY), sX = pow2(eX), limY = pow2(15 - eY), limX = pow2(15 - eX);

  float4 ry[8], rx[XR];
  auto load_rows = [&](int r0, int i0, int i1) {
#pragma unroll
    for (int i = 0; i < 8; ++i) {
      if (i < i0 || i >= i1) continue;
      if (lean_y) {
        const size_t row = (size_t)min(r0 + 8 * rblk + i, R - 1);
        ry[i] = *reinterpret_cast<const float4*>(L.Y + row * 4);
        if ((i & 3) == 0) rg[i >> 2] = *reinterpret_cast<const float4*>(gate3 + row * 128 + c4 * 4);
      } else {
        ry[i] = *reinterpret_cast<const float4*>(L.Y + (size_t)min(r0 + 8 * rblk + i, R - 1) * 128 + c4 * 4);
      }
      if (i < XR && !(lean_x && (i & 3) != 0))
        rx[i] = *reinterpret_cast<const float4*>(L.X + (size_t)min(r0 + xrow + i, R - 1) * KX + xc4 * 4);
    }
  };
  auto rebuild = [&]() {
    if (lean_y) {
      const float4 w0 = *reinterpret_cast<const float4*>(wls + c4 * 4), w1 = *reinterpret_cast<const float4*>(wls + 128 + c4 * 4),
                   w2 = *reinterpret_cast<const float4*>(wls + 256 + c4 * 4), w3 = *reinterpret_cast<const float4*>(wls + 384 + c4 * 4);
#pragma unroll
      for (int i = 0; i < 8; ++i) {
        const float4 g = ry[i], q = rg[i >> 2];
        const float y0 = fmaf(g.w, w3.x, fmaf(g.z, w2.x, fmaf(g.y, w1.x, g.x * w0.x)));
        const float y1 = fmaf(g.w, w3.y, fmaf(g.z, w2.y, fmaf(g.y, w1.y, g.x * w0.y)));
        const float y2 = fmaf(g.w, w3.z, fmaf(g.z, w2.z, fmaf(g.y, w1.z, g.x * w0.z)));
        const float y3 = fmaf(g.w, w3.w, fmaf(g.z, w2.w, fmaf(g.y, w1.w, g.x * w0.w)));
        ry[i] = make_float4(q.x > 0.f ? y0 : 0.f, q.y > 0.f ? y1 : 0.f, q.z > 0.f ? y2 : 0.f, q.w > 0.f ? y3 : 0.f);
      }
    }
    if (lean_x) {
      const float4 a = *reinterpret_cast<const float4*>(wls + c4 * 12), b = *reinterpret_cast<const float4*>(wls + c4 * 12 + 4),
                   c = *reinterpret_cast<const float4*>(wls + c4 * 12 + 8);
      const float wl[12] = {a.x, a.y, a.z, a.w, b.x, b.y, b.z, b.w, c.x, c.y, c.z, c.w};
#pragma unroll
      for (int s = 0; s < 8; s += 4) {
        const float4 p = rx[s];
#pragma unroll
        for (int t = 0; t < 3; ++t)
          rx[s + 1 + t] = make_float4(p.x > 0.f ? wl[t] : 0.f, p.y > 0.f ? wl[3 + t] : 0.f, p.z > 0.f ? wl[6 + t] : 0.f,
                                      p.w > 0.f ? wl[9 + t] : 0.f);
      }
    }
  };
  auto mask = [&](const WgsUnit& u) {
    if (u.r0 + TILE_ROWS > u.rend) {
      const float4 z = make_float4(0.f, 0.f, 0.f, 0.f);
#pragma unroll
      for (int i = 0; i < 8; ++i) if (u.r0 + 8 * rblk + i >= u.rend) ry[i] = z;
#pragma unroll
      for (int i = 0; i < XR; ++i) if (u.r0 + xrow + i >= u.rend) rx[i] = z;
    }
  };
  auto check = [&](float2* set) {
    float my = 0.f, mx = 0.f;
#pragma unroll
    for (int i = 0; i < 8; ++i) my = fmaxf(my, amax4(ry[i]));
#pragma unroll
    for (int i = 0; i < XR; ++i) mx = fmaxf(mx, amax4(rx[i]));
    float py = 0.f, px = 0.f;
    if (__builtin_amdgcn_ballot_w64(my > limY) != 0ull) py = wave_max(my);
    if (__builtin_amdgcn_ballot_w64(mx > limX) != 0ull) px = wave_max(mx);
    if (lane == 0) set[wid] = make_float2(py, px);
  };
  auto adopt = [&](const float2* set) -> int {
    const float4 a = *reinterpret_cast<const float4*>(set), b = *reinterpret_cast<const float4*>(set + 2);
    const float my = fmaxf(fmaxf(a.x, a.z), fmaxf(b.x, b.z)), mx = fmaxf(fmaxf(a.y, a.w), fmaxf(b.y, b.w));
    if (!(my > 0.f) && !(mx > 0.f)) return 0;
    int d = 0, changed = 0;
    if (my > 0.f) { const int e = scale_exp(my) - 2; d += e - eY; eY = e; changed |= 1; }
    if (mx > 0.f) { const int e = scale_exp(mx) - 2; d += e - eX; eX = e; changed |= 2; }
    sY = pow2(eY); sX = pow2(eX); limY = pow2(15 - eY); limX = pow2(15 - eX);
    const float f = pow2(d);
#pragma unroll
    for (int t = 0; t < 2; ++t)
#pragma unroll
      for (int u = 0; u < NB; ++u)
#pragma unroll
        for (int i = 0; i < 16; ++i) acc[t][u][i] *= f;
    return changed;
  };
  auto convert = [&](bool y, bool x) {
    if (y) {
#pragma unroll
      for (int i = 0; i < 8; ++i) tn_store4(Yh, Yl, 8 * rblk + i, c4, ry[i], sY);
    }
    if (x) {
#pragma unroll
      for (int i = 0; i < XR; ++i) tn_store4(Xh, Xl, xrow + i, xc4, rx[i], sX);
    }
  };
  auto frag = [&](const unsigned char* plane, int cb, int ks) { return tn_frag(plane, cb, ks, lane); };

  WgsUnit cur = wgs_unit(0, full, wg, nwg, ntiles, R, rem_rows, q);
  load_rows(cur.r0, 0, 8);
  PP_WAIT_VMEM();
  if (LEAN) rebuild();
  mask(cur);
  check(flags + 4);
  __syncthreads();
  adopt(flags + 4);
  for (int k = 0; k < nunits; ++k) {
    const bool has_next = k + 1 < nunits;
    const WgsUnit nxt = has_next ? wgs_unit(k + 1, full, wg, nwg, ntiles, R, rem_rows, q) : cur;
    if (k > 0) {
      PP_WAIT_VMEM();
      if (LEAN) rebuild();
      mask(cur);
    }
    check(flags);
    convert(true, true);
    if (bias) {
#pragma unroll
      for (int i = 0; i < 8; i += CSTEP) { bsum[0] += ry[i].x; bsum[1] += ry[i].y; bsum[2] += ry[i].z; bsum[3] += ry[i].w; }
    }
    __syncthreads();
    {
      const int changed = adopt(flags);
      if (changed) {
        convert(changed & 1, changed & 2);
        __syncthreads();
      }
    }
    const int ng = (min(cur.rend - cur.r0, TILE_ROWS) + 15) >> 4;
    pp_half8 fa[2][4], fb[2][2 * NB];
    auto fetch = [&](int par, int ks) {
#pragma unroll
      for (int t = 0; t < 2; ++t) { fa[par][2 * t] = frag(Yh, wr * 64 + t * 32, ks); fa[par][2 * t + 1] = frag(Yl, wr * 64 + t * 32, ks); }
#pragma unroll
      for (int u = 0; u < NB; ++u) { fb[par][2 * u] = frag(Xh, 32 * NB * wc + u * 32, ks); fb[par][2 * u + 1] = frag(Xl, 32 * NB * wc + u * 32, ks); }
    };
    fetch(0, 0);
#pragma unroll
    for (int s4 = 0; s4 < TILE_ROWS / 16; ++s4) {
      const int par = s4 & 1;
      if (s4 + 1 < ng) fetch(par ^ 1, (s4 + 1) * 16);
#pragma unroll
      for (int t = 0; t < 2; ++t) {
        if (s4 < ng) {
#pragma unroll
          for (int u = 0; u < NB; ++u) {
            acc[t][u] = __builtin_amdgcn_mfma_f32_32x32x16_f16(fa[par][2 * t + 1], fb[par][2 * u], acc[t][u], 0, 0, 0);
            acc[t][u] = __builtin_amdgcn_mfma_f32_32x32x16_f16(fa[par][2 * t], fb[par][2 * u + 1], acc[t][u], 0, 0, 0);
            acc[t][u] = __builtin_amdgcn_mfma_f32_32x32x16_f16(fa[par][2 * t], fb[par][2 * u], acc[t][u], 0, 0, 0);
          }
        }
        if (t == 0 && has_next) {
          __builtin_amdgcn_sched_barrier(0);
          load_rows(nxt.r0, 2 * s4, 2 * s4 + 2);
          __builtin_amdgcn_sched_barrier(0);
        }
      }
    }
    __syncthreads();
    cur = nxt;
  }
  const float f = pow2(-(eY + eX));
  if (slot != nullptr) {
    float4* __restrict__ s4 = reinterpret_cast<float4*>(slot) + tid;
#pragma unroll
    for (int t = 0; t < 2; ++t)
#pragma unroll
      for (int u = 0; u < NB; ++u)
#pragma unroll
        for (int qq = 0; qq < 4; ++qq)
          s4[((t * NB + u) * 4 + qq) * 256] = make_float4(acc[t][u][4 * qq] * f, acc[t][u][4 * qq + 1] * f, acc[t][u][4 * qq + 2] * f,
                                                          acc[t][u][4 * qq + 3] * f);
  } else {
#pragma unroll
    for (int t = 0; t < 2; ++t)
#pragma unroll
      for (int u = 0; u < NB; ++u) {
        const int k = 32 * NB * wc + u * 32 + l31;
#pragma unroll
        for (int reg = 0; reg < 16; ++reg) {
          const int n = wr * 64 + t * 32 + (reg & 3) + 8 * (reg >> 2) + 4 * lh;
          atomicAdd(&L.Wbar[(size_t)n * KX + k], acc[t][u][reg] * f);
        }
      }
  }
  if (bias) {
    float* red = reinterpret_cast<float*>(img);
#pragma unroll
    for (int j = 0; j < 4; ++j) red[rblk * 128 + c4 * 4 + j] = bsum[j];
    __syncthreads();
    if (tid < 128) {
      float sum = 0.f;
#pragma unroll
      for (int i = 0; i < 8; ++i) sum += red[i * 128 + tid];
      if (slot != nullptr) slot[ORD_WGRAD_BIAS + tid] = sum;
      else atomicAdd(&L.bbar[tid], sum);
    }
  }
}

}

template <int KXC, int CSTEP, bool LEAN>
__global__ __launch_bounds__(256, 2) void k_wgrad_chain_s(WgradOperands LA, WgradOperands LB, WgradOperands LC,
                                                          const int32_t* __restrict__ count, int rmul, int rcap, int nwg_ab, int nwg_c,
                                                          float* __restrict__ part, WgradLean Z) {
  __shared__ __attribute__((aligned(1024))) unsigned char img[4 * TILE_ROWS * 256];
  __shared__ __attribute__((aligned(16))) float2 flags[8];
  __shared__ __attribute__((aligned(16))) float wls[LEAN ? 512 : 4];
  const int R = min(count[0] * rmul, rcap);
  const int ntiles = (R + TILE_ROWS - 1) / TILE_ROWS;
  wgs_active(ntiles, nwg_ab, nwg_c);
  const int bx = blockIdx.x;
  if (bx >= 2 * nwg_ab + nwg_c) return;
  const int layer = bx < nwg_ab ? 0 : (bx < 2 * nwg_ab ? 1 : 2);
  const int wg = bx - layer * nwg_ab, nwg = layer < 2 ? nwg_ab : nwg_c;
  const WgradOperands L = layer == 0 ? LA : (layer == 1 ? LB : LC);
  float* const slot = part != nullptr ? part + (size_t)bx * ORD_WGRAD_SLOT : nullptr;
  if (LEAN) {
    if (layer == 0) { wls[threadIdx.x] = Z.w4[threadIdx.x]; wls[256 + threadIdx.x] = Z.w4[256 + threadIdx.x]; }
    else if (layer == 2) { wls[threadIdx.x] = Z.w0[threadIdx.x]; if (threadIdx.x < 128) wls[256 + threadIdx.x] = Z.w0[256 + threadIdx.x]; }
    __syncthreads();
  }
  if (KXC == 128 || layer < 2) wgs_layer<128, CSTEP, LEAN>(L, Z.gate3, wls, layer, R, ntiles, wg, nwg, img, flags, slot);
  else wgs_layer<KXC, CSTEP, false>(L, Z.gate3, wls, layer, R, ntiles, wg, nwg, img, flags, slot);
}

template <int KXC>
__global__ __launch_bounds__(ORD_RED_THREADS) void k_wgrad_reduce_s(WgradOperands LA, WgradOperands LB, WgradOperands LC,
                                                                    const int32_t* __restrict__ count, int rmul, int rcap, int nwg_ab,
                                                                    int nwg_c, const float* __restrict__ part) {
  __shared__ float4 lds[ORD_RED_GROUPS * 64];
  const int R = min(count[0] * rmul, rcap);
  const int ntiles = (R + TILE_ROWS - 1) / TILE_ROWS;
  wgs_active(ntiles, nwg_ab, nwg_c);
  const int layer = blockIdx.y;
  const WgradOperands L = layer == 0 ? LA : (layer == 1 ? LB : LC);
  const int KX = layer < 2 ? 128 : KXC, NB = KX / 64;
  const int row0 = layer * nwg_ab, rows = layer < 2 ? nwg_ab : nwg_c;
  const bool bias_block = blockIdx.x == 64;
  if ((!bias_block && (int)blockIdx.x * 64 >= 32 * KX) || (bias_block && L.bbar == nullptr)) return;
  const int el = threadIdx.x & 63;
  const int e4 = bias_block ? ORD_WGRAD_BIAS / 4 + el : blockIdx.x * 64 + el;
  float4 s;
  if (!pp_ordered_rows_sum(reinterpret_cast<const float4*>(part), ORD_WGRAD_SLOT / 4, row0, rows, e4, !bias_block || el < 32, lds, s)) return;
  if (bias_block) {
    float4* b4 = reinterpret_cast<float4*>(L.bbar) + el;
    float4 v = *b4;
    v.x += s.x; v.y += s.y; v.z += s.z; v.w += s.w;
    *b4 = v;
    return;
  }
  const int tid = e4 & 255, qq = (e4 >> 8) & 3, tu = e4 >> 10, u = tu % NB, t = tu / NB;
  const int lane = tid & 63, wid = tid >> 6, wr = wid >> 1, wc = wid & 1, l31 = lane & 31, lh = lane >> 5;
  const int k = 32 * NB * wc + u * 32 + l31, n = wr * 64 + t * 32 + 8 * qq + 4 * lh;
  float* __restrict__ w = L.Wbar + (size_t)n * KX + k;
  w[0] += s.x; w[KX] += s.y; w[2 * KX] += s.z; w[3 * KX] += s.w;
}

int pp_launch_wgrad_chain_s(const float* YA, const float* XA, float* WA, const float* YB, const float* XB, float* WB,
                            const float* YC, const float* XC, float* WC, int kxc, const int32_t* count, int rmul, int rcap,
                            hipStream_t st, float* bA, float* bB, float* bC, float* part, const WgradLean* lean) {
  WgradOperands LA{YA, XA, WA, bA}, LB{YB, XB, WB, bB}, LC{YC, XC, WC, bC};
  const WgradLean Z = lean ? *lean : WgradLean{nullptr, nullptr, nullptr};
  const int ntiles = pp_div_up(rcap, TILE_ROWS);
  const int wgs = 2 * PP_FUSED_WGS;
  int nab = kxc == 128 ? wgs / 3 : (wgs * 4) / 11, nc = kxc == 128 ? wgs / 3 : wgs - 2 * ((wgs * 4) / 11);
  if (nab > ntiles) nab = ntiles;
  if (nc > ntiles) nc = ntiles;
  if (kxc == 128 && lean)
    hipLaunchKernelGGL((k_wgrad_chain_s<128, 4, true>), dim3(2 * nab + nc), dim3(256), 0, st, LA, LB, LC, count, rmul, rcap, nab, nc, part, Z);
  else if (kxc == 128)
    hipLaunchKernelGGL((k_wgrad_chain_s<128, 4, false>), dim3(2 * nab + nc), dim3(256), 0, st, LA, LB, LC, count, rmul, rcap, nab, nc, part, Z);
  else
    hipLaunchKernelGGL((k_wgrad_chain_s<64, 1, false>), dim3(2 * nab + nc), dim3(256), 0, st, LA, LB, LC, count, rmul, rcap, nab, nc, part, Z);
  if (part) {
    if (kxc == 128)
      hipLaunchKernelGGL((k_wgrad_reduce_s<128>), dim3(65, 3), dim3(ORD_RED_THREADS), 0, st, LA, LB, LC, count, rmul, rcap, nab, nc, part);
    else
      hipLaunchKernelGGL((k_wgrad_reduce_s<64>), dim3(65, 3), dim3(ORD_RED_THREADS), 0, st, LA, LB, LC, count, rmul, rcap, nab, nc, part);
  }
  return 0;
}
```

### poseprobe_amd/csrc/pp_ordered.h

```cpp
#pragma once
#include "pp_common.h"

#define ORD_WGRAD_SLOT (128 * 128 + 128)
#define ORD_WGRAD_BIAS (128 * 128)
#define ORD_WARP_THIN 1152
#define ORD_WARP_THIN_N 1028
#define ORD_RGB_THIN 512
#define ORD_RGB_THIN_N 387
#define ORD_GEO_ROW 4
#define ORD_GEO_THREADS 512
#define ORD_RAY_ROW 16

struct OrdLayout {
  int64_t wgrad[2];
  int64_t thin[2];
  int64_t geo, ray, total;
};
static inline OrdLayout pp_ord_layout(int work_groups, int capacity, int n_rays) {
  const int64_t w = work_groups < 16 ? 16 : work_groups;
  OrdLayout L;
  int64_t o = 0;
  L.wgrad[0] = o; o += 2 * w * ORD_WGRAD_SLOT;
  L.wgrad[1] = o; o += 2 * w * ORD_WGRAD_SLOT;
  L.thin[0] = o; o += w * ORD_WARP_THIN;
  L.thin[1] = o; o += w * ORD_RGB_THIN;
  L.geo = o; o += (int64_t)pp_div_up(capacity, ORD_GEO_THREADS) * ORD_GEO_ROW;
  L.ray = o; o += (int64_t)n_rays * ORD_RAY_ROW;
  L.total = o;
  return L;
}

struct OrdSegs {
  int n;
  int end[4];
  int off[4];
};
int pp_launch_ordered_flush(const float* part, int stride, int rows_max, const int32_t* count, int cap, int per, const OrdSegs& segs,
                            float* dst, hipStream_t st);

#ifdef __HIPCC__
#define ORD_RED_THREADS 1024
#define ORD_RED_GROUPS (ORD_RED_THREADS / 64)
__device__ __forceinline__ bool pp_ordered_rows_sum(const float4* __restrict__ part, size_t stride4, int row0, int rows, int e4, bool valid,
                                                    float4* __restrict__ lds , float4& out) {
  const int g = threadIdx.x >> 6, el = threadIdx.x & 63;
  float4 s = make_float4(0.f, 0.f, 0.f, 0.f);
  if (valid) {
    const float4* __restrict__ p = part + (size_t)row0 * stride4 + e4;
    int r = g;
    for (; r + 7 * ORD_RED_GROUPS < rows; r += 8 * ORD_RED_GROUPS) {
      float4 v[8];
#pragma unroll
      for (int i = 0; i < 8; ++i) v[i] = p[(size_t)(r + i * ORD_RED_GROUPS) * stride4];
#pragma unroll
      for (int i = 0; i < 8; ++i) { s.x += v[i].x; s.y += v[i].y; s.z += v[i].z; s.w += v[i].w; }
    }
    float4 v[7];
#pragma unroll
    for (int i = 0; i < 7; ++i) v[i] = r + i * ORD_RED_GROUPS < rows ? p[(size_t)(r + i * ORD_RED_GROUPS) * stride4] : make_float4(0.f, 0.f, 0.f, 0.f);
#pragma unroll
    for (int i = 0; i < 7; ++i)
      if (r + i * ORD_RED_GROUPS < rows) { s.x += v[i].x; s.y += v[i].y; s.z += v[i].z; s.w += v[i].w; }
  }
  lds[g * 64 + el] = s;
  __syncthreads();
  if (g != 0) return false;
  out = lds[el];
#pragma unroll
  for (int i = 1; i < ORD_RED_GROUPS; ++i) {
    const float4 v = lds[i * 64 + el];
    out.x += v.x; out.y += v.y; out.z += v.z; out.w += v.w;
  }
  return valid;
}
#endif
```

### poseprobe_amd/csrc/pp_ordered.hip

```cpp
#include "pp_ordered.h"

__global__ __launch_bounds__(ORD_RED_THREADS) void k_ordered_flush(const float* __restrict__ part, int stride, int rows_max,
                                                                   const int32_t* __restrict__ count, int cap, int per, OrdSegs segs,
                                                                   float* __restrict__ dst) {
  __shared__ float4 lds[ORD_RED_GROUPS * 64];
  const int n = segs.end[segs.n - 1];
  int rows = rows_max;
  if (count) rows = min(rows_max, (min(count[0], cap) + per - 1) / per);
  const int e4 = blockIdx.x * 64 + (threadIdx.x & 63);
  float4 s;
  if (!pp_ordered_rows_sum(reinterpret_cast<const float4*>(part), stride >> 2, 0, rows, e4, 4 * e4 < n, lds, s)) return;
  const float v[4] = {s.x, s.y, s.z, s.w};
#pragma unroll
  for (int c = 0; c < 4; ++c) {
    const int i = 4 * e4 + c;
    if (i >= n) break;
    int seg = 0;
    while (i >= segs.end[seg]) ++seg;
    dst[segs.off[seg] + i - (seg ? segs.end[seg - 1] : 0)] += v[c];
  }
}

int pp_launch_ordered_flush(const float* part, int stride, int rows_max, const int32_t* count, int cap, int per, const OrdSegs& segs,
                            float* dst, hipStream_t st) {
  const int n4 = pp_div_up(segs.end[segs.n - 1], 4);
  hipLaunchKernelGGL(k_ordered_flush, dim3(pp_div_up(n4, 64)), dim3(ORD_RED_THREADS), 0, st, part, stride, rows_max, count, cap, per,
                     segs, dst);
  return 0;
}

extern "C" int pp_ordered_workspace(int32_t work_groups, int32_t capacity, int32_t n_rays, int64_t* bytes) {
  PP_REQUIRE(bytes, "null pointer");
  PP_REQUIRE(work_groups > 0 && work_groups <= 4096 && capacity > 0 && n_rays > 0, "bad sizes (1 <= work_groups <= 4096, capacity > 0, n_rays > 0)");
  *bytes = pp_ord_layout(work_groups, capacity, n_rays).total * (int64_t)sizeof(float);
  return PP_OK;
}

extern "C" int pp_ordered_attach(void* ctx, void* work, int64_t work_bytes, int32_t work_groups, int32_t capacity, int32_t n_rays) {
  PP_REQUIRE(ctx, "null context (the workspace is recorded in a context: create one)");
  PPContext* c = static_cast<PPContext*>(ctx);
  if (!work) {
    c->ord = nullptr;
    c->ord_wgs = c->ord_cap = c->ord_rays = 0;
    return PP_OK;
  }
  PP_REQUIRE(work_groups > 0 && work_groups <= 4096 && capacity > 0 && n_rays > 0, "bad sizes (1 <= work_groups <= 4096, capacity > 0, n_rays > 0)");
  PP_REQUIRE((reinterpret_cast<uintptr_t>(work) & 15) == 0, "work must be 16-byte aligned");
  PP_REQUIRE(work_bytes >= pp_ord_layout(work_groups, capacity, n_rays).total * (int64_t)sizeof(float),
             "work is smaller than pp_ordered_workspace(work_groups, capacity, n_rays)");
  c->ord = static_cast<float*>(work);
  c->ord_wgs = work_groups < 16 ? 16 : work_groups;
  c->ord_cap = capacity;
  c->ord_rays = n_rays;
  return PP_OK;
}
```

Baseline: 1.034 million rays/s.

## Split leftover MLP tiles into half-tiles across two workgroups to balance the tail

New measurement: 1.004 million rays/s. 2.9% lower.

```diff
diff --git a/poseprobe_amd/_lib.py b/poseprobe_amd/_lib.py
--- a/poseprobe_amd/_lib.py
+++ b/poseprobe_amd/_lib.py
@@ -82,7 +82,7 @@
 
 
 OPTION_NAMES = ('mlp_fused', 'grid_chunks', 'nerf_split', 'mlp_split', 'mlp_wgs', 'nerf_chain', 'nerf_chain_nw',
-                'nerf_chain_head', 'mlp_pack', 'warp_lean')
+                'nerf_chain_head', 'mlp_pack', 'warp_lean', 'mlp_half_tail')
 
 
 class Context:
diff --git a/poseprobe_amd/csrc/pp_common.h b/poseprobe_amd/csrc/pp_common.h
--- a/poseprobe_amd/csrc/pp_common.h
+++ b/poseprobe_amd/csrc/pp_common.h
@@ -21,6 +21,7 @@
   PP_OPT_NERF_CHAIN_HEAD,
   PP_OPT_MLP_PACK,
   PP_OPT_WARP_LEAN,
+  PP_OPT_MLP_HALF_TAIL,
   PP_OPT_COUNT
 };
 
diff --git a/poseprobe_amd/csrc/pp_error.hip b/poseprobe_amd/csrc/pp_error.hip
--- a/poseprobe_amd/csrc/pp_error.hip
+++ b/poseprobe_amd/csrc/pp_error.hip
@@ -19,7 +19,7 @@
     {"mlp_fused", 1, 0, 1},          {"grid_chunks", 0, 0, 4096},  {"nerf_split", 1, 0, 1},
     {"mlp_split", 31, 0, 31},        {"mlp_wgs", 0, 0, 4096},      {"nerf_chain", 3, 0, 3},
     {"nerf_chain_nw", 4, 4, 8},      {"nerf_chain_head", 1, 0, 1}, {"mlp_pack", 1, 0, 1},
-    {"warp_lean", 1, 0, 1},
+    {"warp_lean", 1, 0, 1},          {"mlp_half_tail", 1, 0, 1},
 };
 static const struct PPDefaults {
   int v[PP_OPT_COUNT];
diff --git a/poseprobe_amd/csrc/pp_mlp_split.hip b/poseprobe_amd/csrc/pp_mlp_split.hip
--- a/poseprobe_amd/csrc/pp_mlp_split.hip
+++ b/poseprobe_amd/csrc/pp_mlp_split.hip
@@ -217,12 +217,53 @@
 }
 __device__ __forceinline__ float slot_get(const unsigned* slot) { return __uint_as_float(*slot); }
 
+struct TileSched {
+  int nfull, lone_tile, lone_mask;
+  __device__ __forceinline__ TileSched(int ntiles, int half_tail) {
+    const int nwg = gridDim.x, w = blockIdx.x, rem = ntiles % nwg;
+    const bool tail = half_tail != 0 && rem > 0 && 2 * rem <= nwg;
+    nfull = tail ? ntiles - rem : ntiles;
+    lone_tile = tail && w < 2 * rem ? nfull + (w >> 1) : -1;
+    lone_mask = 1 << (w & 1);
+  }
+  __device__ __forceinline__ int first(int& mask) const {
+    if ((int)blockIdx.x < nfull) { mask = 3; return blockIdx.x; }
+    mask = lone_mask;
+    return lone_tile;
+  }
+  __device__ __forceinline__ int next(int tile, int mask, int& nmask) const {
+    nmask = 3;
+    if (mask != 3) return -1;
+    const int t = tile + gridDim.x;
+    if (t < nfull) return t;
+    nmask = lone_mask;
+    return lone_tile;
+  }
+};
+__device__ __forceinline__ bool has_half(int mask, int h) { return (mask >> h) & 1; }
+
+template <int KS = 8, int LD = LDH2, int PL = PLANE, class Hook>
+__device__ __forceinline__ void pipe_stage(bool mm, bool ep, const _Float16* __restrict__ rows, const SplitW& w, f32x16& acc, int l31,
+                                           int lh, Hook hook) {
+  if (mm && ep) {
+    zero16(acc);
+    mma_half<KS, LD, PL>(rows, w, acc, l31, lh, [&](int ks) { hook(ks, std::true_type()); });
+  } else if (mm) {
+    zero16(acc);
+    mma_half<KS, LD, PL>(rows, w, acc, l31, lh, [&](int ks) { hook(ks, std::false_type()); });
+  } else {
+#pragma unroll
+    for (int ks = 0; ks < KS; ++ks) hook(ks, std::true_type());
+  }
+}
+#define PP_IF_EPI(epi) if constexpr (decltype(epi)::value)
+
 }
 
 template <bool PACK, bool LEAN>
 __global__ __launch_bounds__(256) void k_warp_fused_fwd_s(const float* __restrict__ params, const float* __restrict__ pts,
                                                           const int32_t* __restrict__ count, int capacity, float out_range,
-                                                          float* __restrict__ acts, float* __restrict__ out,
+                                                          float* __restrict__ acts, float* __restrict__ out, int half_tail,
                                                           const float* __restrict__ pack) {
   __shared__ __attribute__((aligned(16))) _Float16 At[2][2 * PLANE];
   __shared__ __attribute__((aligned(16))) float W4s[4 * LDA];
@@ -235,7 +276,10 @@
   const int M = min(count[0], capacity);
   const int R = 4 * M;
   const int ntiles = (M + 15) >> 4;
-  if ((int)blockIdx.x >= ntiles) return;
+  const TileSched sched(ntiles, half_tail);
+  int hm, hmn;
+  int tile = sched.first(hm);
+  if (tile < 0) return;
   const int tid = threadIdx.x, lane = tid & 63, wid = tid >> 6;
   const int l31 = lane & 31, lh = lane >> 5;
   const int col = wid * 32 + l31;
@@ -289,18 +333,19 @@
     }
   };
   float pnext = 0.f;
-  if (tid < 48 && (int)blockIdx.x * 48 + tid < M * 3) pnext = pts[blockIdx.x * 48 + tid];
+  if (tid < 48 && tile * 48 + tid < M * 3) pnext = pts[tile * 48 + tid];
   park(0, pnext);
   if (tid < 16) Mx[tid >> 3][tid & 7] = 0u;
   __builtin_amdgcn_s_waitcnt(0);
   __syncthreads();
-  int par = 0;
-  for (int tile = blockIdx.x; tile < ntiles; tile += gridDim.x, par ^= 1) {
+  for (int par = 0; tile >= 0; tile = sched.next(tile, hm, hmn), hm = hmn, par ^= 1) {
     const int s0 = tile * 16, r0 = tile * TILE_ROWS;
+    const bool do0 = has_half(hm, 0), do1 = has_half(hm, 1);
     {
-      const int nt = tile + gridDim.x;
+      int nm;
+      const int nt = sched.next(tile, hm, nm);
       pnext = 0.f;
-      if (tid < 48 && nt < ntiles && nt * 48 + tid < M * 3) pnext = pts[nt * 48 + tid];
+      if (tid < 48 && nt >= 0 && nt * 48 + tid < M * 3) pnext = pts[nt * 48 + tid];
     }
     const bool ok0 = acts != nullptr && r0 + l31 < R, ok1 = acts != nullptr && r0 + 32 + l31 < R;
     float* __restrict__ crow = acts + (acts != nullptr ? (size_t)(r0 + l31) * 128 + fb : 0);
@@ -326,54 +371,64 @@
       acc = __builtin_amdgcn_mfma_f32_32x32x16_f16(a0l, xh, acc, 0, 0, 0);
       acc = __builtin_amdgcn_mfma_f32_32x32x16_f16(a0h, xh, acc, 0, 0, 0);
     };
-    layer0(0, acc0);
-    layer0(1, acc1);
+    if (do0) layer0(0, acc0);
+    if (do1) layer0(1, acc1);
     const float inv0 = pow2(-(ein + ew0)), ninv0 = pow2(-e0);
     HalfEpilogue<4, true> ea;
+    if (do0) {
+      ea.begin(brow(3));
+      ea.all(acc0, inv0, sc0, ok0 && (!LEAN || primal), crow, arow0);
+      slot_max(&Mx[par][0], ea.vmax(ninv0), lane);
+    }
+    __syncthreads();
+    if (tid < 8) Mx[par ^ 1][tid] = 0u;
     ea.begin(brow(3));
-    ea.all(acc0, inv0, sc0, ok0 && (!LEAN || primal), crow, arow0);
-    slot_max(&Mx[par][0], ea.vmax(ninv0), lane);
-    __syncthreads();
-    if (tid < 8) Mx[par ^ 1][tid] = 0u;
-    zero16(acc0);
-    ea.begin(brow(3));
-    mma_half(&At[0][0], w1, acc0, l31, lh, [&](int ks) { ea.step(ks, acc1, inv0, sc0, ok1 && (!LEAN || primal), crow + 32 * 128, arow0 + 32 * LDH2); });
-    slot_max(&Mx[par][1], ea.vmax(ninv0), lane);
+    pipe_stage(do0, do1, &At[0][0], w1, acc0, l31, lh, [&](int ks, auto epi) {
+      PP_IF_EPI(epi) ea.step(ks, acc1, inv0, sc0, ok1 && (!LEAN || primal), crow + 32 * 128, arow0 + 32 * LDH2);
+    });
+    if (do1) slot_max(&Mx[par][1], ea.vmax(ninv0), lane);
     park(par ^ 1, pnext);
     __syncthreads();
     const int e10 = scale_exp(fmaf(slot_get(&Mx[par][0]), l1_1, b1mx));
     const float sc10 = pow2(e10), inv1 = pow2(-(e0 + ew1));
-    zero16(acc1);
     ea.begin(brow(0));
-    mma_half(&At[0][32 * LDH2], w1, acc1, l31, lh, [&](int ks) { ea.step(ks, acc0, inv1, sc10, ok0, crow + LS, arow1); });
-    slot_max(&Mx[par][2], ea.vmax(pow2(-e10)), lane);
+    pipe_stage(do1, do0, &At[0][32 * LDH2], w1, acc1, l31, lh, [&](int ks, auto epi) {
+      PP_IF_EPI(epi) ea.step(ks, acc0, inv1, sc10, ok0, crow + LS, arow1);
+    });
+    if (do0) slot_max(&Mx[par][2], ea.vmax(pow2(-e10)), lane);
     __syncthreads();
     const int e11 = scale_exp(fmaf(slot_get(&Mx[par][1]), l1_1, b1mx));
     const float sc11 = pow2(e11);
-    zero16(acc0);
     ea.begin(brow(0));
-    mma_half(&At[1][0], w2, acc0, l31, lh, [&](int ks) { ea.step(ks, acc1, inv1, sc11, ok1, crow + LS + 32 * 128, arow1 + 32 * LDH2); });
-    slot_max(&Mx[par][3], ea.vmax(pow2(-e11)), lane);
+    pipe_stage(do0, do1, &At[1][0], w2, acc0, l31, lh, [&](int ks, auto epi) {
+      PP_IF_EPI(epi) ea.step(ks, acc1, inv1, sc11, ok1, crow + LS + 32 * 128, arow1 + 32 * LDH2);
+    });
+    if (do1) slot_max(&Mx[par][3], ea.vmax(pow2(-e11)), lane);
     __syncthreads();
     const int e20 = scale_exp(fmaf(slot_get(&Mx[par][2]), l1_2, b2mx));
     const float sc20 = pow2(e20), inv20 = pow2(-(e10 + ew2)), inv21 = pow2(-(e11 + ew2));
-    zero16(acc1);
     ea.begin(brow(1));
-    mma_half(&At[1][32 * LDH2], w2, acc1, l31, lh, [&](int ks) { ea.step(ks, acc0, inv20, sc20, ok0, crow + 2 * LS, arow0); });
+    pipe_stage(do1, do0, &At[1][32 * LDH2], w2, acc1, l31, lh, [&](int ks, auto epi) {
+      PP_IF_EPI(epi) ea.step(ks, acc0, inv20, sc20, ok0, crow + 2 * LS, arow0);
+    });
     __syncthreads();
     const int e21 = scale_exp(fmaf(slot_get(&Mx[par][3]), l1_2, b2mx));
     const float sc21 = pow2(e21);
-    zero16(acc0);
     ea.begin(brow(1));
-    mma_half(&At[0][0], w3, acc0, l31, lh, [&](int ks) { ea.step(ks, acc1, inv21, sc21, ok1, crow + 2 * LS + 32 * 128, arow0 + 32 * LDH2); });
+    pipe_stage(do0, do1, &At[0][0], w3, acc0, l31, lh, [&](int ks, auto epi) {
+      PP_IF_EPI(epi) ea.step(ks, acc1, inv21, sc21, ok1, crow + 2 * LS + 32 * 128, arow0 + 32 * LDH2);
+    });
     __syncthreads();
     HalfEpilogue<4, false> ef;
     const float inv30 = pow2(-(e20 + ew3)), inv31 = pow2(-(e21 + ew3));
-    zero16(acc1);
     ef.begin(brow(2));
-    mma_half(&At[0][32 * LDH2], w3, acc1, l31, lh, [&](int ks) { ef.step(ks, acc0, inv30, 1.f, ok0, crow + 3 * LS, reinterpret_cast<_Float16*>(frow1)); });
-    ef.begin(brow(2));
-    ef.all(acc1, inv31, 1.f, ok1, crow + 3 * LS + 32 * 128, reinterpret_cast<_Float16*>(frow1 + 32 * LDA));
+    pipe_stage(do1, do0, &At[0][32 * LDH2], w3, acc1, l31, lh, [&](int ks, auto epi) {
+      PP_IF_EPI(epi) ef.step(ks, acc0, inv30, 1.f, ok0, crow + 3 * LS, reinterpret_cast<_Float16*>(frow1));
+    });
+    if (do1) {
+      ef.begin(brow(2));
+      ef.all(acc1, inv31, 1.f, ok1, crow + 3 * LS + 32 * 128, reinterpret_cast<_Float16*>(frow1 + 32 * LDA));
+    }
     __syncthreads();
     {
       const float* As1 = reinterpret_cast<const float*>(At[1]);
@@ -400,7 +455,7 @@
       const int row = tid >> 2, o = tid & 3;
       const int idx = ((row >> 2) * 4 + o) * 4 + (row & 3);
       const float sum = (Red[idx] + Red[256 + idx]) + (Red[512 + idx] + Red[768 + idx]);
-      if (r0 + row < R) out[(size_t)r0 * 4 + tid] = (sum + b4) * out_range;
+      if (r0 + row < R && has_half(hm, row >> 5)) out[(size_t)r0 * 4 + tid] = (sum + b4) * out_range;
     }
   }
 }
@@ -414,10 +469,11 @@
                                float* acts, float* out, hipStream_t st, const float* pack, bool lean) {
   const int ntiles = pp_div_up(capacity, 16);
   const int grid = ntiles < PP_FUSED_WGS ? ntiles : PP_FUSED_WGS;
+  const int half_tail = pp_opt(PP_OPT_MLP_HALF_TAIL);
   if (lean)
-    launch_pack_variant(k_warp_fused_fwd_s<true, true>, k_warp_fused_fwd_s<false, true>, grid, st, pack, params, pts, count, capacity, out_range, acts, out);
+    launch_pack_variant(k_warp_fused_fwd_s<true, true>, k_warp_fused_fwd_s<false, true>, grid, st, pack, params, pts, count, capacity, out_range, acts, out, half_tail);
   else
-    launch_pack_variant(k_warp_fused_fwd_s<true, false>, k_warp_fused_fwd_s<false, false>, grid, st, pack, params, pts, count, capacity, out_range, acts, out);
+    launch_pack_variant(k_warp_fused_fwd_s<true, false>, k_warp_fused_fwd_s<false, false>, grid, st, pack, params, pts, count, capacity, out_range, acts, out, half_tail);
   return 0;
 }
 
@@ -523,7 +579,7 @@
                                                           const float* __restrict__ acts, const float* __restrict__ out_grad,
                                                           const int32_t* __restrict__ count, int capacity, float out_range,
                                                           float* __restrict__ ybar, float* __restrict__ params_grad,
-                                                          float* __restrict__ pts_grad, float* __restrict__ part,
+                                                          float* __restrict__ pts_grad, float* __restrict__ part, int half_tail,
                                                           const float* __restrict__ pack) {
   __shared__ __attribute__((aligned(16))) _Float16 At[2][2 * PLANE];
   __shared__ __attribute__((aligned(16))) float XS[TILE_ROWS * 128];
@@ -537,7 +593,10 @@
   const int M = min(count[0], capacity);
   const int R = 4 * M;
   const int ntiles = (M + 15) >> 4;
-  if ((int)blockIdx.x >= ntiles) return;
+  const TileSched sched(ntiles, half_tail);
+  int hm, hmn;
+  int tile = sched.first(hm);
+  if (tile < 0) return;
   const int tid = threadIdx.x, lane = tid & 63, wid = tid >> 6;
   const int l31 = lane & 31, lh = lane >> 5;
   const int col = wid * 32 + l31;
@@ -581,12 +640,13 @@
   }
   float wacc4[4] = {0.f, 0.f, 0.f, 0.f}, bacc4 = 0.f, wacc0[3] = {0.f, 0.f, 0.f}, bacc0 = 0.f;
 
-  auto stage_piece = [&](int t, int b, int i) {
+  auto stage_piece = [&](int t, int b, int i, int mask) {
     const int rn0 = t * TILE_ROWS, sn0 = t * 16;
     if (i < 8) {
       const int rl = 16 * wid + 2 * i;
       const int row = min(rn0 + rl + lh, R - 1);
-      __builtin_amdgcn_global_load_lds(PP_GLOBAL_PTR(X3 + (size_t)row * 128 + l31 * 4), PP_LDS_PTR(&XS[rl * 128]), 16, 0, 0);
+      if (has_half(mask, wid >> 1))
+        __builtin_amdgcn_global_load_lds(PP_GLOBAL_PTR(X3 + (size_t)row * 128 + l31 * 4), PP_LDS_PTR(&XS[rl * 128]), 16, 0, 0);
     } else if (i == 8) {
       const int e = min(sn0 * 16 + tid, M * 16 - 1);
       __builtin_amdgcn_global_load_lds(PP_GLOBAL_PTR(out_grad + e), PP_LDS_PTR(&G[b][wid * 64]), 4, 0, 0);
@@ -595,17 +655,19 @@
       __builtin_amdgcn_global_load_lds(PP_GLOBAL_PTR(pts + e), PP_LDS_PTR(&Ps[b][0]), 4, 0, 0);
     }
   };
-  auto stage_gate_piece = [&](const float* __restrict__ X, int r0, int gb, int i) {
+  auto stage_gate_piece = [&](const float* __restrict__ X, int r0, int gb, int i, int mask) {
     const int prow = 4 * wid + 2 * i;
     const int row = min(r0 + 4 * (prow + lh), R - 1);
-    __builtin_amdgcn_global_load_lds(PP_GLOBAL_PTR(X + (size_t)row * 128 + l31 * 4), PP_LDS_PTR(&GT[gb][prow * 128]), 16, 0, 0);
+    if (has_half(mask, wid >> 1))
+      __builtin_amdgcn_global_load_lds(PP_GLOBAL_PTR(X + (size_t)row * 128 + l31 * 4), PP_LDS_PTR(&GT[gb][prow * 128]), 16, 0, 0);
   };
   auto prepare_grad = [&](int t, int b) {
     float gv = G[b][tid];
     if (t * 16 + (tid >> 4) >= M) { gv = 0.f; G[b][tid] = 0.f; }
     slot_max(&Mx[b][6], fabsf(gv), lane);
   };
-  auto w4_accumulate = [&](int b) {
+  auto w4_accumulate = [&](int b, int mask) {
+    if (!has_half(mask, h0)) return;
     const float* __restrict__ xs = &XS[(h0 * 32) * 128 + j0];
 #pragma unroll 8
     for (int r = 0; r < 32; ++r) {
@@ -627,43 +689,47 @@
     acc = __builtin_amdgcn_mfma_f32_32x32x16_f16(a4h, xh, acc, 0, 0, 0);
   };
   int e3n0 = 0, e3n1 = 0;
-  auto out_layer_bwd = [&](int t, int b) {
+  auto out_layer_bwd = [&](int t, int b, int mask) {
     const float gmx = slot_get(&Mx[b][6]);
     const int eg = scale_exp(gmx);
     const int e3 = scale_exp(gmx * w4l1);
     const float sg = pow2(eg), s3 = pow2(e3), inv = pow2(-(eg + ew4)), n3 = pow2(-e3);
     const int r0 = t * TILE_ROWS;
     f32x16 a0, a1;
-    out_layer(b, 0, sg, a0);
-    out_layer(b, 1, sg, a1);
     HalfEpilogueB<true> eb;
     float* crow = LEAN ? nullptr : ybar + (size_t)(r0 + l31) * 128 + fb;
-    if (LEAN && t * 16 + (tid >> 4) < M) ybar[(size_t)t * 256 + tid] = G[b][tid] * out_range;
-    eb.begin(&XS[(4 * pr) * 128 + fb]);
-    eb.all(a0, inv, s3, r0 + l31 < R, crow, &At[0][l31 * LDH2 + fb]);
-    slot_max(&Mx[b][0], eb.vmax(n3), lane);
-    eb.begin(&XS[(32 + 4 * pr) * 128 + fb]);
-    eb.all(a1, inv, s3, r0 + 32 + l31 < R, LEAN ? nullptr : crow + 32 * 128, &At[0][(32 + l31) * LDH2 + fb]);
-    slot_max(&Mx[b][1], eb.vmax(n3), lane);
+    if (LEAN && t * 16 + (tid >> 4) < M && has_half(mask, tid >> 7)) ybar[(size_t)t * 256 + tid] = G[b][tid] * out_range;
+    if (has_half(mask, 0)) {
+      out_layer(b, 0, sg, a0);
+      eb.begin(&XS[(4 * pr) * 128 + fb]);
+      eb.all(a0, inv, s3, r0 + l31 < R, crow, &At[0][l31 * LDH2 + fb]);
+      slot_max(&Mx[b][0], eb.vmax(n3), lane);
+    }
+    if (has_half(mask, 1)) {
+      out_layer(b, 1, sg, a1);
+      eb.begin(&XS[(32 + 4 * pr) * 128 + fb]);
+      eb.all(a1, inv, s3, r0 + 32 + l31 < R, LEAN ? nullptr : crow + 32 * 128, &At[0][(32 + l31) * LDH2 + fb]);
+      slot_max(&Mx[b][1], eb.vmax(n3), lane);
+    }
     e3n0 = e3; e3n1 = e3;
   };
 
   if (tid < 16) Mx[tid >> 3][tid & 7] = 0u;
 #pragma unroll
-  for (int i = 0; i < 10; ++i) stage_piece(blockIdx.x, 0, i);
+  for (int i = 0; i < 10; ++i) stage_piece(tile, 0, i, hm);
   __builtin_amdgcn_s_waitcnt(0);
   __syncthreads();
-  prepare_grad(blockIdx.x, 0);
+  prepare_grad(tile, 0);
   __syncthreads();
-  w4_accumulate(0);
-  out_layer_bwd(blockIdx.x, 0);
+  w4_accumulate(0, hm);
+  out_layer_bwd(tile, 0, hm);
   __syncthreads();
 
-  int par = 0;
-  for (int tile = blockIdx.x; tile < ntiles; tile += gridDim.x, par ^= 1) {
+  for (int par = 0, tnext; tile >= 0; tile = tnext, hm = hmn, par ^= 1) {
     const int r0 = tile * TILE_ROWS, s0 = tile * 16;
-    const int tnext = tile + gridDim.x;
-    const bool more = tnext < ntiles;
+    tnext = sched.next(tile, hm, hmn);
+    const bool more = tnext >= 0;
+    const bool do0 = has_half(hm, 0), do1 = has_half(hm, 1);
     const bool ok0 = r0 + l31 < R, ok1 = r0 + 32 + l31 < R;
     const int e30 = e3n0, e31 = e3n1;
     float* const crow = ybar + (size_t)(r0 + l31) * 128 + fb;
@@ -675,57 +741,53 @@
     f32x16 acc0, acc1;
     HalfEpilogueB<true> eb;
     if (tid < 7) Mx[par ^ 1][tid] = 0u;
-    zero16(acc0);
-    mma_half(&At[0][0], w3, acc0, l31, lh, [&](int ks) {
-      if (ks < 2) stage_gate_piece(X2, r0, 0, ks);
-      if (more) { stage_piece(tnext, par ^ 1, ks); if (ks < 2) stage_piece(tnext, par ^ 1, 8 + ks); }
+    pipe_stage(do0, true, &At[0][0], w3, acc0, l31, lh, [&](int ks, auto) {
+      if (ks < 2) stage_gate_piece(X2, r0, 0, ks, hm);
+      if (more) { stage_piece(tnext, par ^ 1, ks, hmn); if (ks < 2) stage_piece(tnext, par ^ 1, 8 + ks, hmn); }
     });
     PP_WAIT_VMEM();
     __syncthreads();
     const int e20 = scale_exp(slot_get(&Mx[par][0]) * l1_3), e21 = scale_exp(slot_get(&Mx[par][1]) * l1_3);
     if (more) prepare_grad(tnext, par ^ 1);
-    zero16(acc1);
     eb.begin(grow0);
-    mma_half(&At[0][32 * LDH2], w3, acc1, l31, lh, [&](int ks) {
-      eb.step(ks, acc0, pow2(-(e30 + ew3)), pow2(e20), ok0, crow + LS, arow1);
-      if (ks == 7) { stage_gate_piece(X1, r0, 1, 0); stage_gate_piece(X1, r0, 1, 1); }
-    });
-    slot_max(&Mx[par][2], eb.vmax(pow2(-e20)), lane);
-    __syncthreads();
-    zero16(acc0);
+    pipe_stage(do1, do0, &At[0][32 * LDH2], w3, acc1, l31, lh, [&](int ks, auto epi) {
+      PP_IF_EPI(epi) eb.step(ks, acc0, pow2(-(e30 + ew3)), pow2(e20), ok0, crow + LS, arow1);
+      if (ks == 7) { stage_gate_piece(X1, r0, 1, 0, hm); stage_gate_piece(X1, r0, 1, 1, hm); }
+    });
+    if (do0) slot_max(&Mx[par][2], eb.vmax(pow2(-e20)), lane);
+    __syncthreads();
     eb.begin(grow0 + 8 * 128);
-    mma_half(&At[1][0], w2, acc0, l31, lh, [&](int ks) {
+    pipe_stage(do0, do1, &At[1][0], w2, acc0, l31, lh, [&](int ks, auto epi) {
       if (ks == 5) PP_WAIT_VMEM();
-      eb.step(ks, acc1, pow2(-(e31 + ew3)), pow2(e21), ok1, crow + LS + 32 * 128, arow1 + 32 * LDH2);
-    });
-    slot_max(&Mx[par][3], eb.vmax(pow2(-e21)), lane);
+      PP_IF_EPI(epi) eb.step(ks, acc1, pow2(-(e31 + ew3)), pow2(e21), ok1, crow + LS + 32 * 128, arow1 + 32 * LDH2);
+    });
+    if (do1) slot_max(&Mx[par][3], eb.vmax(pow2(-e21)), lane);
     __syncthreads();
     const int e10 = scale_exp(slot_get(&Mx[par][2]) * l1_2), e11 = scale_exp(slot_get(&Mx[par][3]) * l1_2);
-    zero16(acc1);
     eb.begin(grow1);
-    mma_half(&At[1][32 * LDH2], w2, acc1, l31, lh, [&](int ks) {
-      eb.step(ks, acc0, pow2(-(e20 + ew2)), pow2(e10), ok0, crow + 2 * LS, arow0);
-      if (ks == 7) { stage_gate_piece(X0, r0, 0, 0); stage_gate_piece(X0, r0, 0, 1); }
-    });
-    __syncthreads();
-    zero16(acc0);
+    pipe_stage(do1, do0, &At[1][32 * LDH2], w2, acc1, l31, lh, [&](int ks, auto epi) {
+      PP_IF_EPI(epi) eb.step(ks, acc0, pow2(-(e20 + ew2)), pow2(e10), ok0, crow + 2 * LS, arow0);
+      if (ks == 7) { stage_gate_piece(X0, r0, 0, 0, hm); stage_gate_piece(X0, r0, 0, 1, hm); }
+    });
+    __syncthreads();
     eb.begin(grow1 + 8 * 128);
-    mma_half(&At[0][0], w1, acc0, l31, lh, [&](int ks) {
+    pipe_stage(do0, do1, &At[0][0], w1, acc0, l31, lh, [&](int ks, auto epi) {
       if (ks == 5) PP_WAIT_VMEM();
-      eb.step(ks, acc1, pow2(-(e21 + ew2)), pow2(e11), ok1, crow + 2 * LS + 32 * 128, arow0 + 32 * LDH2);
+      PP_IF_EPI(epi) eb.step(ks, acc1, pow2(-(e21 + ew2)), pow2(e11), ok1, crow + 2 * LS + 32 * 128, arow0 + 32 * LDH2);
     });
     __syncthreads();
     HalfEpilogueB<false> ef;
-    zero16(acc1);
     ef.begin(grow0);
-    mma_half(&At[0][32 * LDH2], w1, acc1, l31, lh, [&](int ks) {
-      ef.step(ks, acc0, pow2(-(e10 + ew1)), 1.f, false, nullptr, reinterpret_cast<_Float16*>(frow1));
-    });
-    ef.begin(grow0 + 8 * 128);
-    ef.all(acc1, pow2(-(e11 + ew1)), 1.f, false, nullptr, reinterpret_cast<_Float16*>(frow1 + 32 * LDA));
+    pipe_stage(do1, do0, &At[0][32 * LDH2], w1, acc1, l31, lh, [&](int ks, auto epi) {
+      PP_IF_EPI(epi) ef.step(ks, acc0, pow2(-(e10 + ew1)), 1.f, false, nullptr, reinterpret_cast<_Float16*>(frow1));
+    });
+    if (do1) {
+      ef.begin(grow0 + 8 * 128);
+      ef.all(acc1, pow2(-(e11 + ew1)), 1.f, false, nullptr, reinterpret_cast<_Float16*>(frow1 + 32 * LDA));
+    }
     __syncthreads();
     const float* As1 = reinterpret_cast<const float*>(At[1]);
-    {
+    if (has_half(hm, h0)) {
       const float* __restrict__ yb = &As1[(4 * h0 * 8) * LDA + j0];
       const float* ps = &Ps[par][h0 * 24];
 #pragma unroll
@@ -757,13 +819,13 @@
       Red[wid * 64 + lane] = d0[0] + d1[0];
     }
     if (more) {
-      w4_accumulate(par ^ 1);
-      out_layer_bwd(tnext, par ^ 1);
+      w4_accumulate(par ^ 1, hmn);
+      out_layer_bwd(tnext, par ^ 1, hmn);
     }
     __syncthreads();
     if (tid < 64) {
       const int s = tid >> 2, i = tid & 3;
-      if (i < 3 && s0 + s < M) {
+      if (i < 3 && s0 + s < M && has_half(hm, s >> 3)) {
         const float v = (Red[tid] + Red[64 + tid]) + (Red[128 + tid] + Red[192 + tid]);
         atomicAdd(&pts_grad[(s0 + s) * 3 + i], v);
       }
@@ -804,15 +866,16 @@
                                float* pts_grad, hipStream_t st, const float* pack, float* part, bool lean) {
   const int ntiles = pp_div_up(capacity, 16);
   const int grid = ntiles < PP_FUSED_WGS ? ntiles : PP_FUSED_WGS;
+  const int half_tail = pp_opt(PP_OPT_MLP_HALF_TAIL);
   if (lean)
     launch_pack_variant(k_warp_fused_bwd_s<true, true>, k_warp_fused_bwd_s<false, true>, grid, st, pack, params, pts, acts, out_grad, count,
-                        capacity, out_range, ybar, params_grad, pts_grad, part);
+                        capacity, out_range, ybar, params_grad, pts_grad, part, half_tail);
   else
     launch_pack_variant(k_warp_fused_bwd_s<true, false>, k_warp_fused_bwd_s<false, false>, grid, st, pack, params, pts, acts, out_grad, count,
-                        capacity, out_range, ybar, params_grad, pts_grad, part);
+                        capacity, out_range, ybar, params_grad, pts_grad, part, half_tail);
   if (part) {
     const OrdSegs segs{4, {512, 896, 1024, ORD_WARP_THIN_N}, {WPF_W4, WPF_W0, WPF_B0, WPF_B4}};
-    pp_launch_ordered_flush(part, ORD_WARP_THIN, grid, count, capacity, 16, segs, params_grad, st);
+    pp_launch_ordered_flush(part, ORD_WARP_THIN, grid, count, capacity, 16, segs, params_grad, st, half_tail);
   }
   return 0;
 }
@@ -860,7 +923,8 @@
   return e;
 }
 
-__device__ __forceinline__ void stage_feat_tile_s(const float* __restrict__ feat, int r0, int R, float* Fs, int wid, int lane) {
+__device__ __forceinline__ void stage_feat_tile_s(const float* __restrict__ feat, int r0, int R, float* Fs, int wid, int lane, int mask) {
+  if (!has_half(mask, wid >> 1)) return;
 #pragma unroll
   for (int i = 0; i < 4; ++i) {
     const int rl = 16 * wid + 4 * i + (lane >> 4);
@@ -876,7 +940,7 @@
 __global__ __launch_bounds__(256) void k_rgb_fused_fwd_s(const float* __restrict__ params, const float* __restrict__ feat,
                                                          const int32_t* __restrict__ count, int capacity,
                                                          const float* __restrict__ logit_add, int add_ld,
-                                                         float* __restrict__ acts, float* __restrict__ rgb,
+                                                         float* __restrict__ acts, float* __restrict__ rgb, int half_tail,
                                                          const float* __restrict__ pack) {
   __shared__ __attribute__((aligned(16))) _Float16 At[2][2 * PLANE];
   __shared__ __attribute__((aligned(16))) float Fs[2][TILE_ROWS * 64];
@@ -889,7 +953,10 @@
   __shared__ __attribute__((aligned(16))) float red4[32];
   const int R = min(count[0], capacity);
   const int ntiles = (R + TILE_ROWS - 1) / TILE_ROWS;
-  if ((int)blockIdx.x >= ntiles) return;
+  const TileSched sched(ntiles, half_tail);
+  int hm, hmn;
+  int tile = sched.first(hm);
+  if (tile < 0) return;
   const int tid = threadIdx.x, lane = tid & 63, wid = tid >> 6;
   const int l31 = lane & 31, lh = lane >> 5;
   const int col = wid * 32 + l31;
@@ -921,21 +988,21 @@
   }
   const float b3 = ((tid & 3) < 3) ? params[RGF_B3 + (tid & 3)] : 0.f;
   if (tid < 16) Mx[tid >> 3][tid & 7] = 0u;
-  stage_feat_tile_s(feat, blockIdx.x * TILE_ROWS, R, Fs[0], wid, lane);
+  stage_feat_tile_s(feat, tile * TILE_ROWS, R, Fs[0], wid, lane, hm);
   __builtin_amdgcn_s_waitcnt(0);
   __syncthreads();
 
-  int par = 0;
-  for (int tile = blockIdx.x; tile < ntiles; tile += gridDim.x, par ^= 1) {
+  for (int par = 0, tnext; tile >= 0; tile = tnext, hm = hmn, par ^= 1) {
     const int r0 = tile * TILE_ROWS;
-    const int tnext = tile + gridDim.x;
+    tnext = sched.next(tile, hm, hmn);
+    const bool do0 = has_half(hm, 0), do1 = has_half(hm, 1);
     const bool ok0 = acts != nullptr && r0 + l31 < R, ok1 = acts != nullptr && r0 + 32 + l31 < R;
     float* __restrict__ crow = acts + (acts != nullptr ? (size_t)(r0 + l31) * 128 + fb : 0);
     _Float16* const arow0 = &At[0][l31 * LDH2 + fb];
     _Float16* const arow1 = &At[1][l31 * LDH2 + fb];
     float* const frow0 = reinterpret_cast<float*>(At[0]) + l31 * LDA + fb;
     PP_WAIT_VMEM();
-    {
+    if (has_half(hm, wid >> 1)) {
       const int row = tid >> 2, qd = tid & 3;
       float4 f[4];
 #pragma unroll
@@ -955,44 +1022,53 @@
       if (qd == 0) Er[row] = er;
       slot_max(&Mx[par][wid >> 1], mx, lane);
     }
-    if (tnext < ntiles) stage_feat_tile_s(feat, tnext * TILE_ROWS, R, Fs[par ^ 1], wid, lane);
+    if (tnext >= 0) stage_feat_tile_s(feat, tnext * TILE_ROWS, R, Fs[par ^ 1], wid, lane, hmn);
     __syncthreads();
     if (tid < 6) Mx[par ^ 1][tid] = 0u;
     f32x16 acc0, acc1;
     HalfEpilogue<1, true> ea;
     const int e00 = scale_exp(fmaf(slot_get(&Mx[par][0]), l1_0, b0mx)), e01 = scale_exp(fmaf(slot_get(&Mx[par][1]), l1_0, b0mx));
     const float inv00 = pow2(-(Er[l31] + ew0)), inv01 = pow2(-(Er[32 + l31] + ew0));
-    zero16(acc0);
-    mma_half<4, FLD, FPL>(&Fh[0], w0, acc0, l31, lh);
-    zero16(acc1);
+    if (do0) {
+      zero16(acc0);
+      mma_half<4, FLD, FPL>(&Fh[0], w0, acc0, l31, lh);
+    }
     ea.begin(&Bs[0][fb]);
-    mma_half<4, FLD, FPL>(&Fh[32 * FLD], w0, acc1, l31, lh, [&](int ks) {
-      ea.step(2 * ks, acc0, inv00, pow2(e00), ok0, crow, arow0);
-      ea.step(2 * ks + 1, acc0, inv00, pow2(e00), ok0, crow, arow0);
-    });
-    slot_max(&Mx[par][2], ea.vmax(pow2(-e00)), lane);
-    __syncthreads();
-    zero16(acc0);
+    pipe_stage<4, FLD, FPL>(do1, do0, &Fh[32 * FLD], w0, acc1, l31, lh, [&](int ks, auto epi) {
+      PP_IF_EPI(epi) {
+        ea.step(2 * ks, acc0, inv00, pow2(e00), ok0, crow, arow0);
+        ea.step(2 * ks + 1, acc0, inv00, pow2(e00), ok0, crow, arow0);
+      }
+    });
+    if (do0) slot_max(&Mx[par][2], ea.vmax(pow2(-e00)), lane);
+    __syncthreads();
     ea.begin(&Bs[0][fb]);
-    mma_half(&At[0][0], w1, acc0, l31, lh, [&](int ks) { ea.step(ks, acc1, inv01, pow2(e01), ok1, crow + 32 * 128, arow0 + 32 * LDH2); });
-    slot_max(&Mx[par][3], ea.vmax(pow2(-e01)), lane);
+    pipe_stage(do0, do1, &At[0][0], w1, acc0, l31, lh, [&](int ks, auto epi) {
+      PP_IF_EPI(epi) ea.step(ks, acc1, inv01, pow2(e01), ok1, crow + 32 * 128, arow0 + 32 * LDH2);
+    });
+    if (do1) slot_max(&Mx[par][3], ea.vmax(pow2(-e01)), lane);
     __syncthreads();
     const int e10 = scale_exp(fmaf(slot_get(&Mx[par][2]), l1_1, b1mx));
-    zero16(acc1);
     ea.begin(&Bs[1][fb]);
-    mma_half(&At[0][32 * LDH2], w1, acc1, l31, lh, [&](int ks) { ea.step(ks, acc0, pow2(-(e00 + ew1)), pow2(e10), ok0, crow + LS, arow1); });
+    pipe_stage(do1, do0, &At[0][32 * LDH2], w1, acc1, l31, lh, [&](int ks, auto epi) {
+      PP_IF_EPI(epi) ea.step(ks, acc0, pow2(-(e00 + ew1)), pow2(e10), ok0, crow + LS, arow1);
+    });
     __syncthreads();
     const int e11 = scale_exp(fmaf(slot_get(&Mx[par][3]), l1_1, b1mx));
-    zero16(acc0);
     ea.begin(&Bs[1][fb]);
-    mma_half(&At[1][0], w2, acc0, l31, lh, [&](int ks) { ea.step(ks, acc1, pow2(-(e01 + ew1)), pow2(e11), ok1, crow + LS + 32 * 128, arow1 + 32 * LDH2); });
+    pipe_stage(do0, do1, &At[1][0], w2, acc0, l31, lh, [&](int ks, auto epi) {
+      PP_IF_EPI(epi) ea.step(ks, acc1, pow2(-(e01 + ew1)), pow2(e11), ok1, crow + LS + 32 * 128, arow1 + 32 * LDH2);
+    });
     __syncthreads();
     HalfEpilogue<1, false> ef;
-    zero16(acc1);
     ef.begin(&Bs[2][fb]);
-    mma_half(&At[1][32 * LDH2], w2, acc1, l31, lh, [&](int ks) { ef.step(ks, acc0, pow2(-(e10 + ew2)), 1.f, ok0, crow + 2 * LS, reinterpret_cast<_Float16*>(frow0)); });
-    ef.begin(&Bs[2][fb]);
-    ef.all(acc1, pow2(-(e11 + ew2)), 1.f, ok1, crow + 2 * LS + 32 * 128, reinterpret_cast<_Float16*>(frow0 + 32 * LDA));
+    pipe_stage(do1, do0, &At[1][32 * LDH2], w2, acc1, l31, lh, [&](int ks, auto epi) {
+      PP_IF_EPI(epi) ef.step(ks, acc0, pow2(-(e10 + ew2)), 1.f, ok0, crow + 2 * LS, reinterpret_cast<_Float16*>(frow0));
+    });
+    if (do1) {
+      ef.begin(&Bs[2][fb]);
+      ef.all(acc1, pow2(-(e11 + ew2)), 1.f, ok1, crow + 2 * LS + 32 * 128, reinterpret_cast<_Float16*>(frow0 + 32 * LDA));
+    }
     __syncthreads();
     {
       const float* As0 = reinterpret_cast<const float*>(At[0]);
@@ -1019,7 +1095,7 @@
       const int row = tid >> 2, o = tid & 3;
       const int idx = ((row >> 2) * 4 + o) * 4 + (row & 3);
       const float sum = (Red[idx] + Red[256 + idx]) + (Red[512 + idx] + Red[768 + idx]);
-      if (o < 3 && r0 + row < R) {
+      if (o < 3 && r0 + row < R && has_half(hm, row >> 5)) {
         const size_t m = (size_t)(r0 + row);
         rgb[m * 3 + o] = pp_sigmoid(sum + b3 + (logit_add ? logit_add[m * add_ld + o] : 0.f));
       }
@@ -1031,7 +1107,8 @@
                               const float* logit_add, int add_ld, float* acts, float* rgb, hipStream_t st, const float* pack) {
   const int ntiles = pp_div_up(capacity, TILE_ROWS);
   const int grid = ntiles < PP_FUSED_WGS ? ntiles : PP_FUSED_WGS;
-  launch_pack_variant(k_rgb_fused_fwd_s<true>, k_rgb_fused_fwd_s<false>, grid, st, pack, params, feat, count, capacity, logit_add, add_ld, acts, rgb);
+  launch_pack_variant(k_rgb_fused_fwd_s<true>, k_rgb_fused_fwd_s<false>, grid, st, pack, params, feat, count, capacity, logit_add, add_ld, acts, rgb,
+                      pp_opt(PP_OPT_MLP_HALF_TAIL));
   return 0;
 }
 
@@ -1041,7 +1118,7 @@
                                                          const int32_t* __restrict__ count, int capacity,
                                                          float* __restrict__ ybar, float* __restrict__ params_grad,
                                                          float* __restrict__ feat_grad, float* __restrict__ logit_grad, int lg_ld,
-                                                         float* __restrict__ part, const float* __restrict__ pack) {
+                                                         float* __restrict__ part, int half_tail, const float* __restrict__ pack) {
   __shared__ __attribute__((aligned(16))) _Float16 At[2][2 * PLANE];
   __shared__ __attribute__((aligned(16))) float XS[TILE_ROWS * 128];
   __shared__ __attribute__((aligned(16))) float GT[TILE_ROWS * 128];
@@ -1051,7 +1128,10 @@
   __shared__ __attribute__((aligned(16))) float red4[32];
   const int R = min(count[0], capacity);
   const int ntiles = (R + TILE_ROWS - 1) / TILE_ROWS;
-  if ((int)blockIdx.x >= ntiles) return;
+  const TileSched sched(ntiles, half_tail);
+  int hm, hmn;
+  int tile = sched.first(hm);
+  if (tile < 0) return;
   const int tid = threadIdx.x, lane = tid & 63, wid = tid >> 6;
   const int l31 = lane & 31, lh = lane >> 5;
   const int col = wid * 32 + l31;
@@ -1090,7 +1170,8 @@
   const int j0 = tid & 127, h0 = tid >> 7;
   float wacc3[3] = {0.f, 0.f, 0.f}, bacc3 = 0.f;
 
-  auto stage_tile = [&](const float* __restrict__ X, int r0, float* dst) {
+  auto stage_tile = [&](const float* __restrict__ X, int r0, float* dst, int mask) {
+    if (!has_half(mask, wid >> 1)) return;
 #pragma unroll
     for (int i = 0; i < 8; ++i) {
       const int rl = 16 * wid + 2 * i;
@@ -1098,16 +1179,16 @@
       __builtin_amdgcn_global_load_lds(PP_GLOBAL_PTR(X + (size_t)row * 128 + l31 * 4), PP_LDS_PTR(dst + rl * 128), 16, 0, 0);
     }
   };
-  auto stage = [&](int t, int b) {
+  auto stage = [&](int t, int b, int mask) {
     const int r0 = t * TILE_ROWS;
-    stage_tile(H2, r0, XS);
+    stage_tile(H2, r0, XS, mask);
     if (wid < 3) {
       const int e = min(r0 * 3 + tid, R * 3 - 1);
       __builtin_amdgcn_global_load_lds(PP_GLOBAL_PTR(rgb + e), PP_LDS_PTR(&RG[b][0][wid * 64]), 4, 0, 0);
       __builtin_amdgcn_global_load_lds(PP_GLOBAL_PTR(rgb_grad + e), PP_LDS_PTR(&RG[b][1][wid * 64]), 4, 0, 0);
     }
   };
-  auto logit_grads = [&](int t, int b) {
+  auto logit_grads = [&](int t, int b, int mask) {
     const int r0 = t * TILE_ROWS;
     float gl = 0.f;
     if (tid < 192) {
@@ -1115,13 +1196,14 @@
       const float r = RG[b][0][tid];
       gl = (r0 + m < R) ? RG[b][1][tid] * r * (1.f - r) : 0.f;
       GL[m * 4 + o] = gl;
-      if (logit_grad && r0 + m < R) logit_grad[(size_t)(r0 + m) * lg_ld + o] = gl;
+      if (logit_grad && r0 + m < R && has_half(mask, m >> 5)) logit_grad[(size_t)(r0 + m) * lg_ld + o] = gl;
     } else {
       GL[(tid - 192) * 4 + 3] = 0.f;
     }
     slot_max(&Mx[b][4], fabsf(gl), lane);
   };
-  auto w3_accumulate = [&]() {
+  auto w3_accumulate = [&](int mask) {
+    if (!has_half(mask, h0)) return;
     const float* __restrict__ xs = &XS[(h0 * 32) * 128 + j0];
 #pragma unroll 8
     for (int r = 0; r < 32; ++r) {
@@ -1132,7 +1214,7 @@
     }
   };
   int e2n = 0;
-  auto out_layer_bwd = [&](int t, int b, _Float16* dst) {
+  auto out_layer_bwd = [&](int t, int b, _Float16* dst, int mask) {
     const float gmx = slot_get(&Mx[b][4]);
     const int eg = scale_exp(gmx);
     const int e2 = scale_exp(gmx * w3l1);
@@ -1142,6 +1224,7 @@
     HalfEpilogueB<true> eb;
 #pragma unroll
     for (int hh = 0; hh < 2; ++hh) {
+      if (!has_half(mask, hh)) continue;
       float4 x = *reinterpret_cast<const float4*>(&GL[(hh * 32 + l31) * 4]);
       if (lh != 0) x = make_float4(0.f, 0.f, 0.f, 0.f);
       pp_half8 xh, xl;
@@ -1159,20 +1242,20 @@
   };
 
   if (tid < 16) Mx[tid >> 3][tid & 7] = 0u;
-  stage(blockIdx.x, 0);
+  stage(tile, 0, hm);
   __builtin_amdgcn_s_waitcnt(0);
   __syncthreads();
-  logit_grads(blockIdx.x, 0);
+  logit_grads(tile, 0, hm);
   __syncthreads();
-  w3_accumulate();
-  out_layer_bwd(blockIdx.x, 0, At[0]);
+  w3_accumulate(hm);
+  out_layer_bwd(tile, 0, At[0], hm);
   __syncthreads();
 
-  int par = 0;
-  for (int tile = blockIdx.x; tile < ntiles; tile += gridDim.x, par ^= 1) {
+  for (int par = 0, tnext; tile >= 0; tile = tnext, hm = hmn, par ^= 1) {
     const int r0 = tile * TILE_ROWS;
-    const int tnext = tile + gridDim.x;
-    const bool more = tnext < ntiles;
+    tnext = sched.next(tile, hm, hmn);
+    const bool more = tnext >= 0;
+    const bool do0 = has_half(hm, 0), do1 = has_half(hm, 1);
     const bool ok0 = r0 + l31 < R, ok1 = r0 + 32 + l31 < R;
     _Float16* const Aa = At[par];
     _Float16* const Ab = At[par ^ 1];
@@ -1181,40 +1264,46 @@
     f32x16 acc0, acc1;
     HalfEpilogueB<true> eb;
     if (tid < 5) Mx[par ^ 1][tid] = 0u;
-    if (more) stage(tnext, par ^ 1);
-    stage_tile(H1, r0, GT);
-    zero16(acc0);
-    mma_half(Aa, w2, acc0, l31, lh);
+    if (more) stage(tnext, par ^ 1, hmn);
+    stage_tile(H1, r0, GT, hm);
+    if (do0) {
+      zero16(acc0);
+      mma_half(Aa, w2, acc0, l31, lh);
+    }
     PP_WAIT_VMEM();
     __syncthreads();
     const int e10 = scale_exp(slot_get(&Mx[par][0]) * l1_2), e11 = scale_exp(slot_get(&Mx[par][1]) * l1_2);
-    zero16(acc1);
     eb.begin(&GT[l31 * 128 + fb]);
-    mma_half(Aa + 32 * LDH2, w2, acc1, l31, lh, [&](int ks) {
-      eb.step(ks, acc0, pow2(-(e2 + ew2)), pow2(e10), ok0, crow + LS, Ab + l31 * LDH2 + fb);
-    });
-    slot_max(&Mx[par][2], eb.vmax(pow2(-e10)), lane);
-    __syncthreads();
-    zero16(acc0);
+    pipe_stage(do1, do0, Aa + 32 * LDH2, w2, acc1, l31, lh, [&](int ks, auto epi) {
+      PP_IF_EPI(epi) eb.step(ks, acc0, pow2(-(e2 + ew2)), pow2(e10), ok0, crow + LS, Ab + l31 * LDH2 + fb);
+    });
+    if (do0) slot_max(&Mx[par][2], eb.vmax(pow2(-e10)), lane);
+    __syncthreads();
     eb.begin(&GT[(32 + l31) * 128 + fb]);
-    mma_half(Ab, w1, acc0, l31, lh, [&](int ks) {
-      eb.step(ks, acc1, pow2(-(e2 + ew2)), pow2(e11), ok1, crow + LS + 32 * 128, Ab + (32 + l31) * LDH2 + fb);
-    });
-    slot_max(&Mx[par][3], eb.vmax(pow2(-e11)), lane);
-    __syncthreads();
-    stage_tile(H0, r0, GT);
-    zero16(acc1);
-    mma_half(Ab + 32 * LDH2, w1, acc1, l31, lh);
+    pipe_stage(do0, do1, Ab, w1, acc0, l31, lh, [&](int ks, auto epi) {
+      PP_IF_EPI(epi) eb.step(ks, acc1, pow2(-(e2 + ew2)), pow2(e11), ok1, crow + LS + 32 * 128, Ab + (32 + l31) * LDH2 + fb);
+    });
+    if (do1) slot_max(&Mx[par][3], eb.vmax(pow2(-e11)), lane);
+    __syncthreads();
+    stage_tile(H0, r0, GT, hm);
+    if (do1) {
+      zero16(acc1);
+      mma_half(Ab + 32 * LDH2, w1, acc1, l31, lh);
+    }
     PP_WAIT_VMEM();
     __syncthreads();
     const int e00 = scale_exp(slot_get(&Mx[par][2]) * l1_1), e01 = scale_exp(slot_get(&Mx[par][3]) * l1_1);
-    eb.begin(&GT[l31 * 128 + fb]);
-    eb.all(acc0, pow2(-(e10 + ew1)), pow2(e00), ok0, crow + 2 * LS, Aa + l31 * LDH2 + fb);
-    eb.begin(&GT[(32 + l31) * 128 + fb]);
-    eb.all(acc1, pow2(-(e11 + ew1)), pow2(e01), ok1, crow + 2 * LS + 32 * 128, Aa + (32 + l31) * LDH2 + fb);
-    if (more) logit_grads(tnext, par ^ 1);
-    __syncthreads();
-    {
+    if (do0) {
+      eb.begin(&GT[l31 * 128 + fb]);
+      eb.all(acc0, pow2(-(e10 + ew1)), pow2(e00), ok0, crow + 2 * LS, Aa + l31 * LDH2 + fb);
+    }
+    if (do1) {
+      eb.begin(&GT[(32 + l31) * 128 + fb]);
+      eb.all(acc1, pow2(-(e11 + ew1)), pow2(e01), ok1, crow + 2 * LS + 32 * 128, Aa + (32 + l31) * LDH2 + fb);
+    }
+    if (more) logit_grads(tnext, par ^ 1, hmn);
+    __syncthreads();
+    if (has_half(hm, rb)) {
       f32x16 fa;
       zero16(fa);
       mma_half(Aa + rb * 32 * LDH2, w0, fa, l31, lh);
@@ -1228,8 +1317,8 @@
       }
     }
     if (more) {
-      w3_accumulate();
-      out_layer_bwd(tnext, par ^ 1, Ab);
+      w3_accumulate(hmn);
+      out_layer_bwd(tnext, par ^ 1, Ab, hmn);
     }
     __syncthreads();
   }
@@ -1259,11 +1348,12 @@
                               float* logit_grad, int lg_ld, hipStream_t st, const float* pack, float* part) {
   const int ntiles = pp_div_up(capacity, TILE_ROWS);
   const int grid = ntiles < PP_FUSED_WGS ? ntiles : PP_FUSED_WGS;
+  const int half_tail = pp_opt(PP_OPT_MLP_HALF_TAIL);
   launch_pack_variant(k_rgb_fused_bwd_s<true>, k_rgb_fused_bwd_s<false>, grid, st, pack, params, acts, rgb, rgb_grad, count, capacity, ybar,
-                      params_grad, feat_grad, logit_grad, lg_ld, part);
+                      params_grad, feat_grad, logit_grad, lg_ld, part, half_tail);
   if (part) {
     const OrdSegs segs{2, {384, ORD_RGB_THIN_N, 0, 0}, {RGF_W3, RGF_B3, 0, 0}};
-    pp_launch_ordered_flush(part, ORD_RGB_THIN, grid, count, capacity, TILE_ROWS, segs, params_grad, st);
+    pp_launch_ordered_flush(part, ORD_RGB_THIN, grid, count, capacity, TILE_ROWS, segs, params_grad, st, half_tail);
   }
   return 0;
 }
diff --git a/poseprobe_amd/csrc/pp_ordered.h b/poseprobe_amd/csrc/pp_ordered.h
--- a/poseprobe_amd/csrc/pp_ordered.h
+++ b/poseprobe_amd/csrc/pp_ordered.h
@@ -36,7 +36,7 @@
   int off[4];
 };
 int pp_launch_ordered_flush(const float* part, int stride, int rows_max, const int32_t* count, int cap, int per, const OrdSegs& segs,
-                            float* dst, hipStream_t st);
+                            float* dst, hipStream_t st, int half_tail = 0);
 
 #ifdef __HIPCC__
 #define ORD_RED_THREADS 1024
diff --git a/poseprobe_amd/csrc/pp_ordered.hip b/poseprobe_amd/csrc/pp_ordered.hip
--- a/poseprobe_amd/csrc/pp_ordered.hip
+++ b/poseprobe_amd/csrc/pp_ordered.hip
@@ -2,11 +2,14 @@
 
 __global__ __launch_bounds__(ORD_RED_THREADS) void k_ordered_flush(const float* __restrict__ part, int stride, int rows_max,
                                                                    const int32_t* __restrict__ count, int cap, int per, OrdSegs segs,
-                                                                   float* __restrict__ dst) {
+                                                                   float* __restrict__ dst, int half_tail) {
   __shared__ float4 lds[ORD_RED_GROUPS * 64];
   const int n = segs.end[segs.n - 1];
   int rows = rows_max;
-  if (count) rows = min(rows_max, (min(count[0], cap) + per - 1) / per);
+  if (count) {
+    const int tiles = (min(count[0], cap) + per - 1) / per;
+    rows = tiles >= rows_max ? rows_max : (half_tail && 2 * tiles <= rows_max ? 2 * tiles : tiles);
+  }
   const int e4 = blockIdx.x * 64 + (threadIdx.x & 63);
   float4 s;
   if (!pp_ordered_rows_sum(reinterpret_cast<const float4*>(part), stride >> 2, 0, rows, e4, 4 * e4 < n, lds, s)) return;
@@ -22,10 +25,10 @@
 }
 
 int pp_launch_ordered_flush(const float* part, int stride, int rows_max, const int32_t* count, int cap, int per, const OrdSegs& segs,
-                            float* dst, hipStream_t st) {
+                            float* dst, hipStream_t st, int half_tail) {
   const int n4 = pp_div_up(segs.end[segs.n - 1], 4);
   hipLaunchKernelGGL(k_ordered_flush, dim3(pp_div_up(n4, 64)), dim3(ORD_RED_THREADS), 0, st, part, stride, rows_max, count, cap, per,
-                     segs, dst);
+                     segs, dst, half_tail);
   return 0;
 }
 
```
